# wuxiyang1996/iPLAN

Hardware: AMD Instinct MI355X
Metric: env-steps/sec (whole node), Hetero-Highway chaotic 5-agent (higher is better)
Workload: dtype f32; 1 GPU; Highway chaotic full iPLAN (Behaviour + GAT + soft update), 5 agents x 55 entities, 32 envs/GPU x 90 steps; step = 8 rollouts, each followed by insert + Behavior_policy.learn + Prediction_policy.learn, then IPPOLearner.train (15 epochs x 255 x 90 rows x 5 agents); envs_per_gpu=32

## Files before the change

iplan_amd/csrc/behavior_learn.hip:

```cpp
#define IPLAN_SPLIT_PAIRS
#include <cstdlib>

#include "api_util.h"
#include "gru_tile.h"

namespace iplan {

constexpr int DHd = 64, DT = 4;
constexpr int EHd = 32, ET = 2;
constexpr int DLD = DHd + 8;
constexpr int ELDB = EHd + 8;
constexpr int SVD = IPLAN_BEH_SAVE_DEC, SVE = IPLAN_BEH_SAVE_ENC, SVL = IPLAN_BEH_SAVE_LAT;
constexpr int DSD = IPLAN_BEH_DSAVE_DEC, DSL = IPLAN_BEH_DSAVE_LAT;
constexpr float BEPS = 1e-10f;
constexpr int DEC_FWD_BIAS = 64 + 192 + 192 + 16;
constexpr int SD_X = 0, SD_U = 32, SD_R = 96, SD_Z = 160, SD_N = 224, SD_HN = 288, SD_H = 352, SD_A = 416, SD_Y = 480;
constexpr int DD_DY = 0, DD_DU = 16, DD_DR = 80, DD_DZ = 144, DD_DNI = 208, DD_DNH = 272;
constexpr int SE_U = 0, SE_R = 32, SE_Z = 64, SE_N = 96, SE_HN = 128, SE_H = 160;

__device__ __forceinline__ float chain_sum_b(float v) {
    v += __shfl_xor(v, 1);
    v += __shfl_xor(v, 2);
    v += __shfl_xor(v, 4);
    v += __shfl_xor(v, 8);
    return v;
}

__device__ __forceinline__ int beh_windows(const IplanBehArgs& a) { return a.hard ? a.T / a.L - 1 : a.T - 1 - a.L; }
__device__ __forceinline__ int beh_x_step(const IplanBehArgs& a, int j, int t) { return a.hard ? j * a.L + t : j - (a.L - 1) + t; }
__device__ __forceinline__ int beh_y_step(const IplanBehArgs& a, int j, int t) { return a.hard ? (j + 1) * a.L + t : j + 1 + t; }
__device__ __forceinline__ int beh_m_step(const IplanBehArgs& a, int j, int t) { return a.hard ? j * a.L + t : j + 1 + t; }

__device__ __forceinline__ uint32_t keep_hash(uint64_t seed, uint64_t idx) {
    uint32_t x = (uint32_t)idx ^ ((uint32_t)(idx >> 32) * 0x9E3779B9u) ^ (uint32_t)seed;
    x ^= x >> 16; x *= 0x85EBCA6Bu; x ^= x >> 13; x *= 0xC2B2AE35u; x ^= x >> 16;
    x ^= (uint32_t)(seed >> 32);
    x ^= x >> 15; x *= 0x2C1B3C6Du; x ^= x >> 12;
    return x;
}
__device__ __forceinline__ f32x4 keep_flags4(uint64_t seed, uint64_t base, float p) {
    const uint32_t thr = (uint32_t)(p * 65536.0f);
    const uint32_t h0 = keep_hash(seed, base), h1 = keep_hash(seed, base + 2);
    f32x4 k;
    k[0] = (h0 & 0xFFFFu) >= thr ? 1.0f : 0.0f;
    k[1] = (h0 >> 16) >= thr ? 1.0f : 0.0f;
    k[2] = (h1 & 0xFFFFu) >= thr ? 1.0f : 0.0f;
    k[3] = (h1 >> 16) >= thr ? 1.0f : 0.0f;
    return k;
}

__device__ __forceinline__ f32x4 keep_tile(const IplanBehArgs& a, int net, int j, int row, int t, int T, bool valid, int rows) {
    const int l = lane_id(), g = l >> 4;
    const int64_t base = ((((int64_t)net * beh_windows(a) + j) * rows + row) * a.L + t) * DHd + 16 * T + 4 * g;
    f32x4 k = splat4(0.f);
    if (!valid) return k;
    if (a.keep) {
        for (int q = 0; q < 4; ++q) k[q] = (float)a.keep[base + q];
    } else if (a.drop_p > 0.f) {
        k = keep_flags4(a.seed, (uint64_t)base, a.drop_p);
    } else {
        k = splat4(1.0f);
    }
    return k;
}

__device__ __forceinline__ float window_mask_sum(const IplanBehArgs& a, int net, int j) {
    if (a.win_norm) return a.win_norm[(int64_t)net * beh_windows(a) + j] * (float)(a.N * a.d);
    float s = 0.f;
    const int span = a.hard ? beh_windows(a) * a.L : a.L;
    const int first = a.hard ? 0 : j + 1;
    const int cnt = a.E * span;
    for (int i = lane_id(); i < cnt; i += 64) {
        const int e = i / span, t = i - e * span;
        s += a.mask[((int64_t)net * a.E + e) * a.T + first + t];
    }
    return wave_sum(s) * (float)(a.N * a.d);
}

__device__ __forceinline__ f32x4 ld_row_raw(const float* __restrict__ row, int dim, int g) {
    f32x4 v;
    for (int q = 0; q < 4; ++q) {
        const int i = 4 * g + q;
        v[q] = row[i < dim ? i : dim - 1];
    }
    return v;
}
struct BehChain {
    int net, rows, tiles, tile, row, e, ent, J, n, g;
    bool valid;
    const float* hrow;
    const float* mrow;
    int64_t grow;
};
__device__ __forceinline__ bool beh_chain(const IplanBehArgs& a, BehChain& c) {
    const int l = lane_id();
    c.n = l & 15;
    c.g = l >> 4;
    c.net = (int)blockIdx.y;
    c.rows = a.E * a.N;
    c.tiles = (c.rows + 15) / 16;
    c.tile = (int)blockIdx.x * 4 + (wave_id() & 3);
    c.row = c.tile * 16 + c.n;
    c.valid = c.tile < c.tiles && c.row < c.rows;
    c.e = c.valid ? c.row / a.N : 0;
    c.ent = c.valid ? c.row % a.N : 0;
    c.J = beh_windows(a);
    c.hrow = a.hist ? a.hist + (int64_t)c.net * a.h_s_net + (int64_t)c.e * a.h_s_e + (int64_t)c.ent * a.d : nullptr;
    c.mrow = a.mask ? a.mask + ((int64_t)c.net * a.E + c.e) * a.T : nullptr;
    c.grow = (int64_t)c.net * c.rows + (c.valid ? c.row : 0);
    return c.tile < c.tiles;
}

template <bool BF3>
__global__ __launch_bounds__(256) void beh_enc_fwd_kernel(IplanBehArgs a) {
    __shared__ __attribute__((aligned(16))) float s_wih[BF3 ? 16 : 3 * EHd * ELDB];
    __shared__ __attribute__((aligned(16))) float s_whh[BF3 ? 16 : 3 * EHd * ELDB];
    __shared__ __attribute__((aligned(16))) float s_lin[EHd * 24];
    __shared__ __attribute__((aligned(16))) float s_out[16 * ELDB];
    __shared__ __attribute__((aligned(16))) float s_b[32 + 96 + 96 + 16];
    const float* __restrict__ PE = a.enc_params + (int64_t)blockIdx.y * a.enc_s_net;
    if (!BF3) {
        stage_matrix(s_wih, ELDB, 3 * EHd, PE + a.enc_off[IPLAN_ENC_WIH], 3 * EHd, EHd);
        stage_matrix(s_whh, ELDB, 3 * EHd, PE + a.enc_off[IPLAN_ENC_WHH], 3 * EHd, EHd);
    }
    stage_matrix(s_lin, 24, EHd, PE + a.enc_off[IPLAN_ENC_LIN_W], EHd, a.d);
    stage_matrix(s_out, ELDB, 16, PE + a.enc_off[IPLAN_ENC_OUT_W], a.Z, EHd);
    stage_vector(s_b, 32, PE + a.enc_off[IPLAN_ENC_LIN_B], 32);
    stage_vector(s_b + 32, 96, PE + a.enc_off[IPLAN_ENC_BIH], 96);
    stage_vector(s_b + 128, 96, PE + a.enc_off[IPLAN_ENC_BHH], 96);
    stage_vector(s_b + 224, 16, PE + a.enc_off[IPLAN_ENC_OUT_B], a.Z);
    __syncthreads();
    BehChain c;
    if (!beh_chain(a, c)) return;
    const bool valid = c.valid;
    const int g = c.g, J = c.J, l = lane_id();
    const int j_lo = imax(a.fwd_j_lo, 0), j_hi = a.fwd_j_hi > 0 ? imin(a.fwd_j_hi, J) : J;
    float* carry = a.enc_carry ? a.enc_carry + ((int64_t)c.net * c.tiles + c.tile) * 768 : nullptr;
    f32x4 he[ET], lat = splat4(0.f);
    for (int t = 0; t < ET; ++t) he[t] = splat4(0.f);
    if (j_lo > 0 && carry) {
        for (int t = 0; t < ET; ++t) he[t] = *reinterpret_cast<const f32x4*>(carry + 256 * t + 4 * l);
        lat = *reinterpret_cast<const f32x4*>(carry + 512 + 4 * l);
    }
    auto x_fetch = [&](int j, int t, bool& has) {
        const int st = beh_x_step(a, j, t);
        has = st >= 0;
        return ld_row_raw(c.hrow + (int64_t)(st < 0 ? 0 : st) * a.h_s_t, a.d, g);
    };
    bool x_has = false;
    f32x4 x_raw = x_fetch(j_lo, 0, x_has);
    const int64_t ecgs = (int64_t)J * a.L * 256;
    float* enc_rec = a.saved_enc + ((int64_t)c.net * c.tiles + (c.tile < c.tiles ? c.tile : 0)) * (SVE / 16) * ecgs + 16 * c.n;
    Bf3 wih[BF3 ? 6 : 1], whh[BF3 ? 6 : 1];
    f32x4 b_rz[4], b_in[2], b_hn[2];
    if (BF3) {
        for (int t = 0; t < 6; ++t) {
            wih[t] = wfrag_bf3(PE + a.enc_off[IPLAN_ENC_WIH], EHd, 3 * EHd, 16 * t, 0);
            whh[t] = wfrag_bf3(PE + a.enc_off[IPLAN_ENC_WHH], EHd, 3 * EHd, 16 * t, 0);
        }
        for (int t = 0; t < 4; ++t) b_rz[t] = bfrag_lds(s_b + 32, t) + bfrag_lds(s_b + 128, t);
        for (int t = 0; t < 2; ++t) { b_in[t] = bfrag_lds(s_b + 32, 4 + t); b_hn[t] = bfrag_lds(s_b + 128, 4 + t); }
    }
    for (int j = j_lo; j < j_hi; ++j) {
        float* sl = a.saved_lat + (c.grow * J + j) * SVL;
        vstore_a(sl + 16, valid, 0, lat);
        for (int t = 0; t < a.L; ++t) {
            f32x4 x1[1];
            for (int q = 0; q < 4; ++q) x1[0][q] = keep_if(valid && x_has && 4 * g + q < a.d, x_raw[q]);
            {
                const bool last_t = t + 1 == a.L, more = j + 1 < j_hi;
                x_raw = x_fetch(last_t && more ? j + 1 : j, last_t ? (more ? 0 : t) : t + 1, x_has);
            }
            float* se = enc_rec + ((int64_t)j * a.L + t) * 256;
            f32x4 ue[ET];
            for (int T = 0; T < ET; ++T) {
                ue[T] = relu4(dense_tile<1>(s_lin, 24, 16 * T, x1, bfrag_lds(s_b, T)));
                vstore_a(se + ((SE_U >> 4) + T) * ecgs, valid, 0, ue[T]);
            }
            GruGates ke[ET];
            if (BF3) {
                const Bf3 us = split_bf3(ue[0], ue[1]), hs = split_bf3(he[0], he[1]);
                f32x4 acc[6] = {b_rz[0], b_rz[1], b_rz[2], b_rz[3], b_in[0], b_in[1]}, ahn[2] = {b_hn[0], b_hn[1]};
#define ENC_BF3_ROUND(WP, XP)                                                          \
    for (int cc = 0; cc < 6; ++cc) acc[cc] = mfma_bf16(wih[cc].WP, us.XP, acc[cc]);
                ENC_BF3_ROUND(p2, p0) ENC_BF3_ROUND(p0, p2) ENC_BF3_ROUND(p1, p1) ENC_BF3_ROUND(p1, p0) ENC_BF3_ROUND(p0, p1) ENC_BF3_ROUND(p0, p0)
#undef ENC_BF3_ROUND
#define ENC_BF3_ROUND(WP, XP)                                                          \
    for (int cc = 0; cc < 4; ++cc) acc[cc] = mfma_bf16(whh[cc].WP, hs.XP, acc[cc]);    \
    for (int cc = 0; cc < 2; ++cc) ahn[cc] = mfma_bf16(whh[4 + cc].WP, hs.XP, ahn[cc]);
                ENC_BF3_ROUND(p2, p0) ENC_BF3_ROUND(p0, p2) ENC_BF3_ROUND(p1, p1) ENC_BF3_ROUND(p1, p0) ENC_BF3_ROUND(p0, p1) ENC_BF3_ROUND(p0, p0)
#undef ENC_BF3_ROUND
                for (int T = 0; T < ET; ++T) {
                    ke[T] = gru_gates(acc[T], acc[2 + T], acc[4 + T], ahn[T], he[T]);
                    he[T] = ke[T].h;
                }
            } else {
                gru_step_lds<ET, ET>(s_wih, ELDB, s_whh, ELDB, s_b + 32, s_b + 128, ue, he, ke);
            }
            for (int T = 0; T < ET; ++T) {
                vstore_a(se + ((SE_R >> 4) + T) * ecgs, valid, 0, ke[T].r);
                vstore_a(se + ((SE_Z >> 4) + T) * ecgs, valid, 0, ke[T].z);
                vstore_a(se + ((SE_N >> 4) + T) * ecgs, valid, 0, ke[T].n);
                vstore_a(se + ((SE_HN >> 4) + T) * ecgs, valid, 0, ke[T].hn);
                vstore_a(se + ((SE_H >> 4) + T) * ecgs, valid, 0, he[T]);
            }
        }
        const f32x4 lg = dense_tile<ET>(s_out, ELDB, 0, he, bfrag_lds(s_b + 224, 0));
        float mx = -INFINITY;
        for (int q = 0; q < 4; ++q)
            if (4 * g + q < a.Z) mx = fmaxf(mx, lg[q]);
        mx = fmaxf(mx, __shfl_xor(mx, 16));
        mx = fmaxf(mx, __shfl_xor(mx, 32));
        f32x4 ex;
        float ss = 0.f;
        for (int q = 0; q < 4; ++q) { ex[q] = (4 * g + q < a.Z) ? expf(lg[q] - mx) : 0.f; ss += ex[q]; }
        ss = group_sum(ss);
        f32x4 nl;
        for (int q = 0; q < 4; ++q) nl[q] = ex[q] / ss;
        vstore_a(sl, valid, 0, nl);
        for (int q = 0; q < 4; ++q) lat[q] = a.hard ? nl[q] : (1.0f - a.coef) * lat[q] + nl[q] * a.coef;
    }
    if (j_hi < J && carry) {
        for (int t = 0; t < ET; ++t) *reinterpret_cast<f32x4*>(carry + 256 * t + 4 * l) = he[t];
        *reinterpret_cast<f32x4*>(carry + 512 + 4 * l) = lat;
    }
}

constexpr int DEC_TILES = 3;
constexpr int DEC_THREADS = 256 * DEC_TILES;


struct DecTile {
    int net, rows, tiles, tile, J;
    bool live, full, valid;
    int n, g, row, e, ent;
    uint32_t rec_lane;
    const char* hist;
    uint32_t hist_lane;
    const char* mask;
    uint32_t mask_lane;
    int64_t grow0;
    int64_t trow0;
};
__device__ __forceinline__ void dec_tile(const IplanBehArgs& a, DecTile& c, int tile) {
    const int l = lane_id();
    c.n = l & 15;
    c.g = l >> 4;
    c.net = (int)blockIdx.y;
    c.rows = a.E * a.N;
    c.tiles = (c.rows + 15) / 16;
    c.tile = tile;
    c.live = tile < c.tiles;
    c.full = c.live && tile * 16 + 15 < c.rows;
    c.row = tile * 16 + c.n;
    c.valid = c.live && c.row < c.rows;
    const int rr = c.valid ? c.row : 0;
    c.e = rr / a.N;
    c.ent = rr - c.e * a.N;
    c.J = beh_windows(a);
    c.hist = reinterpret_cast<const char*>(a.hist ? a.hist + (int64_t)c.net * a.h_s_net : nullptr);
    c.hist_lane = (uint32_t)(((int64_t)c.e * a.h_s_e + (int64_t)c.ent * a.d) * 4);
    c.mask = reinterpret_cast<const char*>(a.mask ? a.mask + (int64_t)c.net * a.E * a.T : nullptr);
    c.mask_lane = (uint32_t)(c.e * a.T * 4);
    c.grow0 = (int64_t)c.net * c.rows + (int64_t)(c.live ? tile : 0) * 16;
    c.trow0 = ((int64_t)c.net * c.tiles + (int64_t)(c.live ? tile : 0)) * 16;
}

#define REC_CG(col) ((uint32_t)((col) >> 4))

template <bool FULL>
__device__ __forceinline__ f32x4 ld4(const char* __restrict__ base, uint32_t off, bool valid) {
    const f32x4 v = *reinterpret_cast<const f32x4*>(base + ((FULL || valid) ? off : 0u));
    return FULL ? v : zero_unless(valid, v);
}
template <bool FULL>
__device__ __forceinline__ f32x4 ld4_raw(const char* __restrict__ base, uint32_t off, bool valid) {
    return *reinterpret_cast<const f32x4*>(base + ((FULL || valid) ? off : 0u));
}
template <bool FULL>
__device__ __forceinline__ f32x4 ld_row_raw(const char* __restrict__ base, uint32_t off, bool valid, int dim, int g) {
    const uint32_t o = (FULL || valid) ? off : 0u;
    f32x4 v;
    for (int q = 0; q < 4; ++q) {
        const int i = 4 * g + q;
        v[q] = *reinterpret_cast<const float*>(base + (o + 4u * (uint32_t)(i < dim ? i : dim - 1)));
    }
    return v;
}
template <bool FULL>
__device__ __forceinline__ void st4(char* __restrict__ base, uint32_t off, bool valid, f32x4 v) {
    if (FULL || valid) *reinterpret_cast<f32x4*>(base + off) = v;
}
template <bool FULL>
__device__ __forceinline__ f32x4 ld_row_br(const char* __restrict__ base, uint32_t off, bool valid, int dim, int g) {
    f32x4 v = splat4(0.f);
    if (FULL || valid) {
        const float* p = reinterpret_cast<const float*>(base + off) + 4 * g;
        for (int q = 0; q < 4; ++q)
            if (4 * g + q < dim) v[q] = p[q];
    }
    return v;
}

constexpr int XF_H = 0, XF_U = 4, XF_Y = 8, XF_SLOTS = 11;

template <bool FULL, int Q>
__device__ __forceinline__ void dec_fwd_body(const IplanBehArgs& a, const DecTile& c, const float* __restrict__ s_wih,
                                             const float* __restrict__ s_whh, const float* __restrict__ s_lin,
                                             const float* __restrict__ s_out, const float* __restrict__ s_b, float* __restrict__ xch,
                                             int* __restrict__ tcnt) {
    constexpr int q = Q;
#ifndef DEC_FWD_TILE_SYNC
#define DEC_FWD_TILE_SYNC 0
#endif
#ifndef DEC_BWD_TILE_SYNC
#define DEC_BWD_TILE_SYNC 1
#endif
    int sync_n = 0;
    auto tile_sync = [&]() {
        if (DEC_FWD_TILE_SYNC) { sync_n += 4; IPLAN_TILE_SYNC(tcnt, sync_n); }
        else IPLAN_LDS_BARRIER();
    };
    const bool valid = c.valid;
    const int l = lane_id(), g = c.g, J = c.J, net = c.net;
    const float inv_keep = 1.0f / (1.0f - a.drop_p);
    const bool dec_only = a.win != nullptr;
    const int Lw = a.L;
    auto put = [&](int slot, f32x4 v) { *reinterpret_cast<f32x4*>(xch + slot * 256 + 4 * l) = v; };
    auto get = [&](int slot) { return *reinterpret_cast<const f32x4*>(xch + slot * 256 + 4 * l); };
    const int j_lo = dec_only ? 0 : imax(a.fwd_j_lo, 0), j_hi = (!dec_only && a.fwd_j_hi > 0) ? imin(a.fwd_j_hi, J) : J;
    const int64_t steps_per_chain = (int64_t)J * Lw;
    char* sd_base = reinterpret_cast<char*>(a.saved_dec + c.trow0 * steps_per_chain * SVD);
    const uint32_t sd_lane = 64u * (uint32_t)c.n + 16u * (uint32_t)g, cgs = (uint32_t)(steps_per_chain * 1024);
    const char* sl_base = reinterpret_cast<const char*>(a.saved_lat ? a.saved_lat + c.grow0 * J * SVL : nullptr);
    const uint32_t sl_lane = (uint32_t)((int64_t)c.n * J * SVL * 4);
    float* carry = (a.dec_carry && c.live) ? a.dec_carry + ((int64_t)net * c.tiles + c.tile) * 1024 : nullptr;
    const int64_t grow = c.grow0 + c.n;

    auto latent_shifted = [&](int j) {
        f32x4 v = splat4(0.f);
        if (FULL || valid) {
            const float* lp = dec_only ? a.lat_in + grow * a.Z
                                       : reinterpret_cast<const float*>(sl_base + sl_lane + (uint32_t)j * (uint32_t)(SVL * 4)) + 16;
            for (int k = 0; k < 4; ++k) {
                const int z = 4 * g + k - a.d;
                if (z >= 0 && z < a.Z) v[k] = lp[z];
            }
        }
        return v;
    };
    auto x_of = [&](int j, int t) {
        if (dec_only) return ld_row_br<FULL>(reinterpret_cast<const char*>(a.win), (uint32_t)((grow * Lw + t) * a.d * 4), valid, a.d, g);
        const int st = beh_x_step(a, j, t);
        if (st < 0) return splat4(0.f);
        return ld_row_br<FULL>(c.hist, c.hist_lane + (uint32_t)((int64_t)st * a.h_s_t * 4), valid, a.d, g);
    };
    auto u_own = [&](f32x4 xin) {
        f32x4 x1[1];
        x1[0] = xin;
        return relu4(dense_tile<1>(s_lin, 24, 16 * q, x1, bfrag_lds(s_b, q)));
    };

    f32x4 h[DT], u[DT];
    for (int i = 0; i < DT; ++i) h[i] = dec_only ? ld4<FULL>(reinterpret_cast<const char*>(a.hd_in), (uint32_t)(grow * DHd * 4) + 64u * i + 16u * g, valid)
                                                 : splat4(0.f);
    if (j_lo > 0 && carry)
        for (int i = 0; i < DT; ++i) h[i] = *reinterpret_cast<const f32x4*>(carry + 256 * i + 4 * l);
    f32x4 latsh = latent_shifted(j_lo);
    f32x4 xin = x_of(j_lo, 0) + latsh;
    put(XF_U + q, u_own(xin));
    tile_sync();
    for (int i = 0; i < DT; ++i) u[i] = get(XF_U + i);
    tile_sync();

    float beh = 0.f, stab = 0.f;
    const int rows3[3] = {16 * q, DHd + 16 * q, 2 * DHd + 16 * q};
    for (int j = j_lo; j < j_hi; ++j) {
        const float scale = (dec_only || q) ? 0.f : (float)(a.d * a.N) / (window_mask_sum(a, net, j) + BEPS);
        float err = 0.f;
        f32x4 latsh_next = latsh;
        if (j + 1 < j_hi) latsh_next = latent_shifted(j + 1);
        for (int t = 0; t < Lw; ++t) {
            const uint32_t so = sd_lane + (uint32_t)(((int64_t)j * Lw + t) * 1024);
            const bool last_t = t + 1 == Lw;
            const bool has_next = !last_t || j + 1 < j_hi;
            f32x4 xin_next = splat4(0.f);
            if (has_next) xin_next = x_of(last_t ? j + 1 : j, last_t ? 0 : t + 1) + (last_t ? latsh_next : latsh);
            f32x4 nx = splat4(0.f);
            float m = 0.f;
            if (q == 0 && !dec_only) {
                nx = ld_row_br<FULL>(c.hist, c.hist_lane + (uint32_t)((int64_t)beh_y_step(a, j, t) * a.h_s_t * 4), valid, a.d, g);
                if (FULL || valid) m = *reinterpret_cast<const float*>(c.mask + c.mask_lane + 4u * (uint32_t)beh_m_step(a, j, t));
            }
            if (q == 0) st4<FULL>(sd_base, so + cgs * REC_CG(SD_X), valid, xin);
            st4<FULL>(sd_base, so + cgs * REC_CG(SD_U + 16 * q), valid, u[q]);
            f32x4 ai[3], ah[3];
            ai[0] = bfrag_lds(s_b + 64, q) + bfrag_lds(s_b + 256, q);
            ai[1] = bfrag_lds(s_b + 64, DT + q) + bfrag_lds(s_b + 256, DT + q);
            ai[2] = bfrag_lds(s_b + 64, 2 * DT + q);
            dense_multi<3, DT>(s_wih, DLD, rows3, 0, u, ai);
            ah[0] = ai[0];
            ah[1] = ai[1];
            ah[2] = bfrag_lds(s_b + 256, 2 * DT + q);
            dense_multi<3, DT>(s_whh, DLD, rows3, 0, h, ah);
            const GruGates o = gru_gates(ah[0], ah[1], ai[2], ah[2], h[q]);
            st4<FULL>(sd_base, so + cgs * REC_CG(SD_R + 16 * q), valid, o.r);
            st4<FULL>(sd_base, so + cgs * REC_CG(SD_Z + 16 * q), valid, o.z);
            st4<FULL>(sd_base, so + cgs * REC_CG(SD_N + 16 * q), valid, o.n);
            st4<FULL>(sd_base, so + cgs * REC_CG(SD_HN + 16 * q), valid, o.hn);
            st4<FULL>(sd_base, so + cgs * REC_CG(SD_H + 16 * q), valid, o.h);
            const f32x4 km = keep_tile(a, net, j, c.row, t, q, FULL || valid, c.rows);
            f32x4 act[1];
            for (int k = 0; k < 4; ++k) act[0][k] = tanh_f(o.h[k]) * (km[k] * inv_keep);
            st4<FULL>(sd_base, so + cgs * REC_CG(SD_A + 16 * q), valid, act[0]);
            const f32x4 yp = dense_tile_k<1>(s_out, DLD, 0, 16 * q, act, q ? splat4(0.f) : bfrag_lds(s_b + 448, 0));
            put(XF_H + q, o.h);
            if (q) put(XF_Y + q - 1, yp);
            if (has_next) put(XF_U + q, u_own(xin_next));
            tile_sync();
            for (int i = 0; i < DT; ++i) h[i] = (i == q) ? o.h : get(XF_H + i);
            if (has_next)
                for (int i = 0; i < DT; ++i) u[i] = get(XF_U + i);
            f32x4 y = yp;
            if (q == 0) y = (yp + get(XF_Y)) + (get(XF_Y + 1) + get(XF_Y + 2));
            tile_sync();
            const f32x4 xt = xin;
            xin = xin_next;
            if (q) continue;
            st4<FULL>(sd_base, so + cgs * REC_CG(SD_Y), valid, y);
            if (dec_only) {
                if (FULL || valid) {
                    float* po = a.pred_out + (grow * Lw + t) * a.d + 4 * g;
                    for (int k = 0; k < 4; ++k)
                        if (4 * g + k < a.d) po[k] = y[k];
                }
                continue;
            }
            float d2 = 0.f;
            for (int k = 0; k < 4; ++k) {
                if (4 * g + k < a.d) {
                    err += fabsf(nx[k] - y[k]) * m;
                    const float df = xt[k] - y[k];
                    d2 = fmaf(df, df, d2);
                }
            }
            d2 = group_sum(d2);
            if ((FULL || valid) && g == 0) stab += fmaxf(sqrtf(d2) - a.thres, 0.f);
        }
        latsh = latsh_next;
        if (dec_only) {
            st4<FULL>(reinterpret_cast<char*>(a.hd_out), (uint32_t)(grow * DHd * 4) + 64u * q + 16u * g, valid, h[q]);
            return;
        }
        beh = fmaf(err, scale, beh);
    }
    if (j_hi < J && carry) *reinterpret_cast<f32x4*>(carry + 256 * q + 4 * l) = h[q];
    beh = chain_sum_b(group_sum(beh)) / (a.hard ? 1.0f : (float)J);
    stab = chain_sum_b(group_sum(stab)) / (float)a.E / (float)a.L / (float)J;
    if (l == 0 && q == 0 && c.live) {
        float* lp = a.loss_part + ((int64_t)net * c.tiles + c.tile) * 2;
        lp[0] = j_lo > 0 ? lp[0] + beh : beh;
        lp[1] = j_lo > 0 ? lp[1] + stab : stab;
    }
}

__global__ __launch_bounds__(DEC_THREADS) void beh_dec_fwd_kernel(IplanBehArgs a) {
    IPLAN_DYN_LDS(smem);
    float* s_wih = smem;
    float* s_whh = s_wih + 3 * DHd * DLD;
    float* s_lin = s_whh + 3 * DHd * DLD;
    float* s_out = s_lin + DHd * 24;
    float* s_b = s_out + 16 * DLD;
    float* s_xch = s_b + DEC_FWD_BIAS;
    int* s_tcnt = reinterpret_cast<int*>(s_xch + DEC_TILES * XF_SLOTS * 256);
    if (threadIdx.x < 16) s_tcnt[threadIdx.x] = 0;
    const float* __restrict__ PD = a.dec_params + (int64_t)blockIdx.y * a.dec_s_net;
    stage_matrix(s_wih, DLD, 3 * DHd, PD + a.dec_off[IPLAN_DEC_WIH], 3 * DHd, DHd);
    stage_matrix(s_whh, DLD, 3 * DHd, PD + a.dec_off[IPLAN_DEC_WHH], 3 * DHd, DHd);
    stage_matrix(s_lin, 24, DHd, PD + a.dec_off[IPLAN_DEC_LIN_W], DHd, a.d + a.Z);
    stage_matrix(s_out, DLD, 16, PD + a.dec_off[IPLAN_DEC_OUT_W], a.d, DHd);
    stage_vector(s_b, 64, PD + a.dec_off[IPLAN_DEC_LIN_B], 64);
    stage_vector(s_b + 64, 192, PD + a.dec_off[IPLAN_DEC_BIH], 192);
    stage_vector(s_b + 256, 192, PD + a.dec_off[IPLAN_DEC_BHH], 192);
    stage_vector(s_b + 448, 16, PD + a.dec_off[IPLAN_DEC_OUT_B], a.d);
    __syncthreads();
    const int w = uniform_i(wave_id()), q = w & 3, ts = w >> 2;
    DecTile c;
    dec_tile(a, c, (int)blockIdx.x * DEC_TILES + ts);
    float* xch = s_xch + ts * (XF_SLOTS * 256);
#define IPLAN_DEC_FWD(F, QQ) dec_fwd_body<F, QQ>(a, c, s_wih, s_whh, s_lin, s_out, s_b, xch, s_tcnt + ts)
    if (c.full) { if (q == 0) IPLAN_DEC_FWD(true, 0); else if (q == 1) IPLAN_DEC_FWD(true, 1); else if (q == 2) IPLAN_DEC_FWD(true, 2); else IPLAN_DEC_FWD(true, 3); }
    else { if (q == 0) IPLAN_DEC_FWD(false, 0); else if (q == 1) IPLAN_DEC_FWD(false, 1); else if (q == 2) IPLAN_DEC_FWD(false, 2); else IPLAN_DEC_FWD(false, 3); }
#undef IPLAN_DEC_FWD
}

__global__ __launch_bounds__(64) void beh_loss_kernel(IplanBehArgs a) {
    const int net = (int)blockIdx.x;
    const int tiles = (a.E * a.N + 15) / 16;
    float b = 0.f, s = 0.f;
    for (int i = lane_id(); i < tiles; i += 64) {
        b += a.loss_part[((int64_t)net * tiles + i) * 2];
        s += a.loss_part[((int64_t)net * tiles + i) * 2 + 1];
    }
    b = wave_sum(b);
    s = wave_sum(s);
    if (lane_id() == 0) {
        a.loss[net * 2] = b;
        a.loss[net * 2 + 1] = s;
    }
}

constexpr int XB_SLOTS = 16;

template <bool FULL, int Q>
__device__ __forceinline__ void dec_bwd_body(const IplanBehArgs& a, const DecTile& c, const float* __restrict__ s_wihT,
                                             const float* __restrict__ s_whhT, const float* __restrict__ s_outT,
                                             const float* __restrict__ s_latT, float* __restrict__ xch, int* __restrict__ tcnt) {
    constexpr int TLD = 3 * DHd + 8;
    int sync_n = 0;
    auto tile_sync = [&]() {
        if (DEC_BWD_TILE_SYNC) { sync_n += 4; IPLAN_TILE_SYNC(tcnt, sync_n); }
        else IPLAN_LDS_BARRIER();
    };
    const bool valid = c.valid;
    const int l = lane_id(), g = c.g, J = c.J, net = c.net, Lw = a.L;
    const float inv_keep = 1.0f / (1.0f - a.drop_p);
    auto put = [&](int slot, f32x4 v) { *reinterpret_cast<f32x4*>(xch + slot * 256 + 4 * l) = v; };
    auto get = [&](int slot) { return *reinterpret_cast<const f32x4*>(xch + slot * 256 + 4 * l); };
    const int64_t steps_per_chain = (int64_t)J * Lw;
    const char* sd_base = reinterpret_cast<const char*>(a.saved_dec + c.trow0 * steps_per_chain * SVD);
    const uint32_t sd_lane = 64u * (uint32_t)c.n + 16u * (uint32_t)g, cgs = (uint32_t)(steps_per_chain * 1024);
    char* dd_base = reinterpret_cast<char*>(a.dsave_dec + c.trow0 * steps_per_chain * DSD);
    const uint32_t dd_lane = sd_lane;
    char* dl_base = reinterpret_cast<char*>(a.dsave_lat + c.grow0 * J * DSL);
    const uint32_t dl_lane = (uint32_t)((int64_t)c.n * J * DSL * 4) + 16u * (uint32_t)g;

    struct StepIn {
        f32x4 r, z, n, hn, hp, u, y, nx, xc;
        float m;
        bool first, has_xc;
    };
    auto load_step = [&](int j, int t, StepIn& o) {
        const uint32_t so = sd_lane + (uint32_t)(((int64_t)j * Lw + t) * 1024);
        o.first = (j == 0 && t == 0);
        o.r = ld4_raw<FULL>(sd_base, so + cgs * REC_CG(SD_R + 16 * Q), valid);
        o.z = ld4_raw<FULL>(sd_base, so + cgs * REC_CG(SD_Z + 16 * Q), valid);
        o.n = ld4_raw<FULL>(sd_base, so + cgs * REC_CG(SD_N + 16 * Q), valid);
        o.hn = ld4_raw<FULL>(sd_base, so + cgs * REC_CG(SD_HN + 16 * Q), valid);
        o.u = ld4_raw<FULL>(sd_base, so + cgs * REC_CG(SD_U + 16 * Q), valid);
        o.hp = ld4_raw<FULL>(sd_base, (o.first ? so : so - 1024u) + cgs * REC_CG(SD_H + 16 * Q), valid);
        o.y = ld4_raw<FULL>(sd_base, so + cgs * REC_CG(SD_Y), valid);
        o.nx = ld_row_raw<FULL>(c.hist, c.hist_lane + (uint32_t)((int64_t)beh_y_step(a, j, t) * a.h_s_t * 4), valid, a.d, g);
        o.m = *reinterpret_cast<const float*>(c.mask + c.mask_lane + 4u * (uint32_t)beh_m_step(a, j, t));
        o.has_xc = false;
        o.xc = splat4(0.f);
        if (a.penalty != 0.f) {
            const int st = beh_x_step(a, j, t);
            o.has_xc = st >= 0;
            o.xc = ld_row_raw<FULL>(c.hist, c.hist_lane + (uint32_t)((int64_t)(st < 0 ? 0 : st) * a.h_s_t * 4), valid, a.d, g);
        }
    };
    auto mask_step = [&](StepIn& o) {
        o.hp = zero_unless(!o.first, o.hp);
        for (int k = 0; k < 4; ++k) o.xc[k] = keep_if(o.has_xc && 4 * g + k < a.d, o.xc[k]);
        if (!FULL) {
            o.r = zero_unless(valid, o.r); o.z = zero_unless(valid, o.z); o.n = zero_unless(valid, o.n);
            o.hn = zero_unless(valid, o.hn); o.u = zero_unless(valid, o.u); o.hp = zero_unless(valid, o.hp);
            o.y = zero_unless(valid, o.y); o.nx = zero_unless(valid, o.nx); o.xc = zero_unless(valid, o.xc);
            o.m = keep_if(valid, o.m);
        }
    };
    const float pen = a.penalty / (float)J / (float)(a.E_norm > 0 ? a.E_norm : a.E) / (float)Lw;
    const int j_hi = a.bwd_j_hi > 0 ? imin(a.bwd_j_hi, J) : J, j_lo = imax(a.bwd_j_lo, 0);
    float* carry = (a.dec_carry && c.live) ? a.dec_carry + ((int64_t)net * c.tiles + c.tile) * 1024 + 256 * Q : nullptr;
    f32x4 dhd = (j_hi < J && carry) ? *reinterpret_cast<const f32x4*>(carry + 4 * l) : splat4(0.f);
    StepIn cur;
    load_step(j_hi - 1, Lw - 1, cur);
    f32x4 hcur = ld4<FULL>(sd_base, sd_lane + (uint32_t)((((int64_t)(j_hi - 1)) * Lw + (Lw - 1)) * 1024) + cgs * REC_CG(SD_H + 16 * Q), valid);
    for (int j = j_hi - 1; j >= j_lo; --j) {
        const float scale = (float)(a.d * a.N) / (window_mask_sum(a, net, j) + BEPS) / (a.hard ? 1.0f : (float)J);
        f32x4 dlat = splat4(0.f);
        for (int t = Lw - 1; t >= 0; --t) {
            const uint32_t dof = dd_lane + (uint32_t)(((int64_t)j * Lw + t) * 1024);
            mask_step(cur);
            f32x4 dy[1];
            for (int k = 0; k < 4; ++k) {
                float v = 0.f;
                if ((FULL || valid) && 4 * g + k < a.d) {
                    const float er = cur.nx[k] - cur.y[k];
                    v = -((er > 0.f) ? 1.0f : (er < 0.f ? -1.0f : 0.0f)) * cur.m * scale;
                }
                dy[0][k] = v;
            }
            if (a.penalty != 0.f) {
                float d2 = 0.f;
                f32x4 df;
                for (int k = 0; k < 4; ++k) {
                    df[k] = (4 * g + k < a.d) ? cur.xc[k] - cur.y[k] : 0.f;
                    d2 = fmaf(df[k], df[k], d2);
                }
                const float nrm = sqrtf(group_sum(d2));
                if ((FULL || valid) && nrm > a.thres)
                    for (int k = 0; k < 4; ++k) dy[0][k] -= pen * df[k] / nrm;
            }
#ifndef BWD_ABL
#define BWD_ABL 0
#endif
            if (Q == 0 && BWD_ABL != 1) st4<FULL>(dd_base, dof + cgs * REC_CG(DD_DY), valid, dy[0]);
            const f32x4 da = dense_tile<1>(s_outT, 24, 16 * Q, dy, splat4(0.f));
            const f32x4 km = keep_tile(a, net, j, c.row, t, Q, FULL || valid, c.rows);
            f32x4 dht;
            for (int k = 0; k < 4; ++k) {
                const float th = tanh_f(hcur[k]);
                dht[k] = fmaf(da[k] * km[k] * inv_keep, 1.0f - th * th, dhd[k]);
            }
            const GruGrads o = gru_gates_bwd(dht, cur.r, cur.z, cur.n, cur.hn, cur.hp);
            if (BWD_ABL != 1) {
                st4<FULL>(dd_base, dof + cgs * REC_CG(DD_DR + 16 * Q), valid, o.dr);
                st4<FULL>(dd_base, dof + cgs * REC_CG(DD_DZ + 16 * Q), valid, o.dz);
                st4<FULL>(dd_base, dof + cgs * REC_CG(DD_DNI + 16 * Q), valid, o.dni);
                st4<FULL>(dd_base, dof + cgs * REC_CG(DD_DNH + 16 * Q), valid, o.dnh);
            }
            put(0 * 4 + Q, o.dr);
            put(1 * 4 + Q, o.dz);
            put(2 * 4 + Q, o.dni);
            put(3 * 4 + Q, o.dnh);
            const f32x4 u_own = cur.u;
            hcur = cur.hp;
            IPLAN_SCHED_FENCE();
            if (BWD_ABL != 2) {
                const bool wrap = t == 0, more = j > j_lo;
                load_step(wrap && more ? j - 1 : j, wrap ? (more ? Lw - 1 : 0) : t - 1, cur);
            }
            if (BWD_ABL != 5) tile_sync();
            f32x4 du = splat4(0.f), pd = splat4(0.f);
            auto b_ih = [&](int kt) { const int gate = kt >> 2, T = kt & 3;
                                      return (T == Q) ? (gate == 0 ? o.dr : (gate == 1 ? o.dz : o.dni)) : get(gate * 4 + T); };
            auto b_hn = [&](int T) { return (T == Q) ? o.dnh : get(3 * 4 + T); };
            f32x4 fa = wfrag_lds(s_wihT, TLD, 16 * Q, 0), fb = wfrag_lds(s_whhT, TLD, 16 * Q, 0);
            f32x4 bi = b_ih(0), bh = bi;
#pragma unroll
            for (int kt = 0; kt < 3 * DT; ++kt) {
                f32x4 fan = fa, fbn = fb, bin = bi, bhn = bh;
                if (kt + 1 < 3 * DT) {
                    fan = wfrag_lds(s_wihT, TLD, 16 * Q, 16 * (kt + 1));
                    fbn = wfrag_lds(s_whhT, TLD, 16 * Q, 16 * (kt + 1));
                    bin = b_ih(kt + 1);
                    bhn = (kt + 1) < 2 * DT ? bin : b_hn((kt + 1) & 3);
                }
                if (BWD_ABL != 3)
                    for (int k = 0; k < 4; ++k) {
                        du = mfma4(fa[k], bi[k], du);
                        pd = mfma4(fb[k], bh[k], pd);
                    }
                else { du += fa * bi; pd += fb * bh; }
                fa = fan; fb = fbn; bi = bin; bh = bhn;
            }
            f32x4 dup[1];
            for (int k = 0; k < 4; ++k) dup[0][k] = u_own[k] > 0.f ? du[k] : 0.f;
            if (BWD_ABL != 1) st4<FULL>(dd_base, dof + cgs * REC_CG(DD_DU + 16 * Q), valid, dup[0]);
            dhd = o.dh_direct + pd;
            dlat = dense_tile_k<1>(s_latT, DLD, 0, 16 * Q, dup, dlat);
            if (BWD_ABL != 4) tile_sync();
        }
        if (Q) put(Q - 1, dlat);
        tile_sync();
        if (Q == 0) st4<FULL>(dl_base, dl_lane + (uint32_t)j * (uint32_t)(DSL * 4), valid, (dlat + get(0)) + (get(1) + get(2)));
        tile_sync();
    }
    if (j_lo > 0 && carry) *reinterpret_cast<f32x4*>(carry + 4 * l) = dhd;
}

__global__ __launch_bounds__(DEC_THREADS) void beh_dec_bwd_kernel(IplanBehArgs a) {
    IPLAN_DYN_LDS(smem);
    constexpr int TLD = 3 * DHd + 8;
    float* s_wihT = smem;
    float* s_whhT = s_wihT + DHd * TLD;
    float* s_outT = s_whhT + DHd * TLD;
    float* s_latT = s_outT + DHd * 24;
    float* s_xch = s_latT + 16 * DLD;
    int* s_tcnt = reinterpret_cast<int*>(s_xch + DEC_TILES * XB_SLOTS * 256);
    if (threadIdx.x < 16) s_tcnt[threadIdx.x] = 0;
    const float* __restrict__ PD = a.dec_params + (int64_t)blockIdx.y * a.dec_s_net;
    const int din = a.d + a.Z;
    stage_matrix_t(s_wihT, TLD, DHd, PD + a.dec_off[IPLAN_DEC_WIH], 3 * DHd, DHd);
    stage_matrix_t(s_whhT, TLD, DHd, PD + a.dec_off[IPLAN_DEC_WHH], 3 * DHd, DHd);
    stage_matrix_t(s_outT, 24, DHd, PD + a.dec_off[IPLAN_DEC_OUT_W], a.d, DHd);
    {
        const float* Wl = PD + a.dec_off[IPLAN_DEC_LIN_W];
        for (int idx = (int)threadIdx.x; idx < 16 * DLD; idx += (int)blockDim.x) {
            const int z = idx / DLD, m = idx - z * DLD;
            s_latT[idx] = (z < a.Z && m < DHd) ? Wl[(int64_t)m * din + a.d + z] : 0.f;
        }
    }
    __syncthreads();
    const int w = uniform_i(wave_id()), q = w & 3, ts = w >> 2;
    DecTile c;
    dec_tile(a, c, (int)blockIdx.x * DEC_TILES + ts);
    float* xch = s_xch + ts * (XB_SLOTS * 256);
#define IPLAN_DEC_BWD(F, QQ) dec_bwd_body<F, QQ>(a, c, s_wihT, s_whhT, s_outT, s_latT, xch, s_tcnt + ts)
    if (c.full) { if (q == 0) IPLAN_DEC_BWD(true, 0); else if (q == 1) IPLAN_DEC_BWD(true, 1); else if (q == 2) IPLAN_DEC_BWD(true, 2); else IPLAN_DEC_BWD(true, 3); }
    else { if (q == 0) IPLAN_DEC_BWD(false, 0); else if (q == 1) IPLAN_DEC_BWD(false, 1); else if (q == 2) IPLAN_DEC_BWD(false, 2); else IPLAN_DEC_BWD(false, 3); }
#undef IPLAN_DEC_BWD
}

constexpr int EP_WIH = 0, EP_WHH = 3072, EP_BIH = 6144, EP_BHH = 6240, EP_LINW = 6336, EP_LINB = 6848, EP_OUTW = 6880, EP_OUTB = 7392;
static_assert(IPLAN_BEH_ENC_PART == 7408, "enc_part layout");

constexpr int EB_FRAGS = 2 * 2 * 3;
template <bool BF3>
__global__ __launch_bounds__(256) void beh_enc_bwd_kernel(IplanBehArgs a) {
    constexpr int TLE = 3 * EHd + 8;
    __shared__ __attribute__((aligned(16))) float s_wihT[BF3 ? 16 : EHd * TLE];
    __shared__ __attribute__((aligned(16))) float s_whhT[BF3 ? 16 : EHd * TLE];
    __shared__ __attribute__((aligned(16))) bf16x8 s_wp[BF3 ? EB_FRAGS * 3 * 64 : 1];
    __shared__ __attribute__((aligned(16))) float s_outT[EHd * 24];
    __shared__ __attribute__((aligned(16))) float s_turn[4][15][256];
    const float* __restrict__ PE = a.enc_params + (int64_t)blockIdx.y * a.enc_s_net;
    if (BF3) {
        for (int f = wave_id(); f < EB_FRAGS; f += 4) {
            const int mtx = f / 6, T = (f / 3) & 1, ch = f % 3;
            const Bf3 w = wfrag_t_bf3(PE + a.enc_off[mtx ? IPLAN_ENC_WHH : IPLAN_ENC_WIH], EHd, 16 * T, 32 * ch);
            s_wp[(f * 3 + 0) * 64 + lane_id()] = w.p0;
            s_wp[(f * 3 + 1) * 64 + lane_id()] = w.p1;
            s_wp[(f * 3 + 2) * 64 + lane_id()] = w.p2;
        }
    } else {
        stage_matrix_t(s_wihT, TLE, EHd, PE + a.enc_off[IPLAN_ENC_WIH], 3 * EHd, EHd);
        stage_matrix_t(s_whhT, TLE, EHd, PE + a.enc_off[IPLAN_ENC_WHH], 3 * EHd, EHd);
    }
    stage_matrix_t(s_outT, 24, EHd, PE + a.enc_off[IPLAN_ENC_OUT_W], a.Z, EHd);
    __syncthreads();
    BehChain c;
    const bool live = beh_chain(a, c);
    const bool valid = c.valid;
    const int l = lane_id(), n = c.n, g = c.g, J = c.J;
    float (*turn)[256] = s_turn[wave_id()];
    const float cn = a.hard ? 1.0f : a.coef, ck = a.hard ? 0.0f : 1.0f - a.coef;

    f32x4 aWih[6][2], aWhh[6][2], aLin[2], aOut[2];
    f32x4 bG[8], bU[2], bO;
    for (int t = 0; t < 6; ++t)
        for (int u = 0; u < 2; ++u) { aWih[t][u] = splat4(0.f); aWhh[t][u] = splat4(0.f); }
    for (int u = 0; u < 2; ++u) { aLin[u] = splat4(0.f); aOut[u] = splat4(0.f); bU[u] = splat4(0.f); }
    for (int t = 0; t < 8; ++t) bG[t] = splat4(0.f);
    bO = splat4(0.f);
    auto park = [&](int slot, f32x4 v) { *reinterpret_cast<f32x4*>(&turn[slot][n * 16 + ((4 * g + 4 * (n >> 1)) & 15)]) = v; };
    auto pick = [&](int slot, int s) { const int r = 4 * s + g; return turn[slot][r * 16 + ((n + 4 * (r >> 1)) & 15)]; };

    const int j_hi = a.bwd_j_hi > 0 ? imin(a.bwd_j_hi, J) : J, j_lo = imax(a.bwd_j_lo, 0);
    float* carry = (a.enc_carry && live) ? a.enc_carry + ((int64_t)c.net * c.tiles + c.tile) * 768 : nullptr;
    f32x4 dhe[ET], dlat = splat4(0.f);
    for (int t = 0; t < ET; ++t) dhe[t] = splat4(0.f);
    if (j_hi < J && carry) {
        for (int t = 0; t < ET; ++t) dhe[t] = *reinterpret_cast<const f32x4*>(carry + 256 * t + 4 * l);
        dlat = *reinterpret_cast<const f32x4*>(carry + 512 + 4 * l);
    }
    struct EncIn {
        f32x4 r[ET], z[ET], n[ET], hn[ET], u[ET], hp[ET], x;
        bool first, has_x;
    };
    const bool ok = valid && live;
    const int64_t ecgs = (int64_t)J * a.L * 256;
    const float* rec0 = a.saved_enc + ((int64_t)c.net * c.tiles + (c.tile < c.tiles ? c.tile : 0)) * (SVE / 16) * ecgs + 16 * c.n + 4 * g;
    auto load_step = [&](int j, int t, EncIn& o) {
        const int64_t step = (int64_t)j * a.L + t;
        o.first = step == 0;
        const float* se = rec0 + step * 256;
        const float* sp = o.first ? se : se - 256;
        for (int T = 0; T < ET; ++T) {
            o.hp[T] = *reinterpret_cast<const f32x4*>(sp + ((SE_H >> 4) + T) * ecgs);
            o.u[T] = *reinterpret_cast<const f32x4*>(se + ((SE_U >> 4) + T) * ecgs);
            o.r[T] = *reinterpret_cast<const f32x4*>(se + ((SE_R >> 4) + T) * ecgs);
            o.z[T] = *reinterpret_cast<const f32x4*>(se + ((SE_Z >> 4) + T) * ecgs);
            o.n[T] = *reinterpret_cast<const f32x4*>(se + ((SE_N >> 4) + T) * ecgs);
            o.hn[T] = *reinterpret_cast<const f32x4*>(se + ((SE_HN >> 4) + T) * ecgs);
        }
        const int st = beh_x_step(a, j, t);
        o.has_x = st >= 0;
        o.x = ld_row_raw(c.hrow + (int64_t)(st < 0 ? 0 : st) * a.h_s_t, a.d, g);
    };
    auto mask_step = [&](EncIn& o) {
        for (int T = 0; T < ET; ++T) {
            o.hp[T] = zero_unless(ok && !o.first, o.hp[T]);
            o.u[T] = zero_unless(ok, o.u[T]);
            o.r[T] = zero_unless(ok, o.r[T]);
            o.z[T] = zero_unless(ok, o.z[T]);
            o.n[T] = zero_unless(ok, o.n[T]);
            o.hn[T] = zero_unless(ok, o.hn[T]);
        }
        for (int q = 0; q < 4; ++q) o.x[q] = keep_if(ok && o.has_x && 4 * g + q < a.d, o.x[q]);
    };
    struct WinIn {
        f32x4 nl, dl, hL[ET];
    };
    auto load_win = [&](int j, WinIn& o) {
        o.nl = *reinterpret_cast<const f32x4*>(a.saved_lat + (c.grow * J + j) * SVL + 4 * g);
        o.dl = *reinterpret_cast<const f32x4*>(a.dsave_lat + (c.grow * J + j) * DSL + 4 * g);
        for (int T = 0; T < ET; ++T) o.hL[T] = *reinterpret_cast<const f32x4*>(rec0 + ((int64_t)j * a.L + (a.L - 1)) * 256 + ((SE_H >> 4) + T) * ecgs);
    };
    EncIn cur;
    WinIn win;
    load_step(j_hi - 1, a.L - 1, cur);
    load_win(j_hi - 1, win);
    for (int j = j_hi - 1; j >= j_lo; --j) {
        f32x4 dlog[1], hL[ET];
        {
            const f32x4 nl = zero_unless(ok && a.Z > 1, win.nl);
            float s = 0.f;
            f32x4 dnew;
            for (int q = 0; q < 4; ++q) { dnew[q] = cn * dlat[q]; s = fmaf(nl[q], dnew[q], s); }
            s = group_sum(s);
            const f32x4 dl_dec = zero_unless(ok, win.dl);
            for (int q = 0; q < 4; ++q) {
                dlog[0][q] = nl[q] * (dnew[q] - s);
                dlat[q] = ck * dlat[q] + dl_dec[q];
                bO[q] += dlog[0][q];
            }
            for (int T = 0; T < ET; ++T) {
                hL[T] = zero_unless(ok, win.hL[T]);
                dhe[T] = dense_tile<1>(s_outT, 24, 16 * T, dlog, dhe[T]);
            }
            park(0, dlog[0]); park(1, hL[0]); park(2, hL[1]);
            IPLAN_WAVE_SYNC();
            for (int s4 = 0; s4 < 4; ++s4) {
                const float av = pick(0, s4);
                aOut[0] = mfma4(av, pick(1, s4), aOut[0]);
                aOut[1] = mfma4(av, pick(2, s4), aOut[1]);
            }
            IPLAN_WAVE_SYNC();
        }
        for (int t = a.L - 1; t >= 0; --t) {
            f32x4 dg[4 * ET], dd[ET], u[ET], hp[ET];
            mask_step(cur);
            for (int T = 0; T < ET; ++T) {
                hp[T] = cur.hp[T];
                u[T] = cur.u[T];
                const GruGrads o = gru_gates_bwd(dhe[T], cur.r[T], cur.z[T], cur.n[T], cur.hn[T], hp[T]);
                dg[T] = o.dr; dg[ET + T] = o.dz; dg[2 * ET + T] = o.dni; dg[3 * ET + T] = o.dnh;
                dd[T] = o.dh_direct;
            }
            for (int k = 0; k < 8; ++k) bG[k] += dg[k];
            const int oe[ET] = {0, 16};
            f32x4 du[ET], dup[ET];
            for (int T = 0; T < ET; ++T) { du[T] = splat4(0.f); dhe[T] = dd[T]; }
            if (BF3) {
                for (int ch = 0; ch < 3; ++ch) {
                    const Bf3 gi = split_bf3(dg[2 * ch], dg[2 * ch + 1]);
                    const Bf3 gh = ch < 2 ? gi : split_bf3(dg[3 * ET], dg[3 * ET + 1]);
                    Bf3 wi[ET], wh[ET];
                    for (int T = 0; T < ET; ++T) {
                        const bf16x8* fi = s_wp + ((0 * 2 + T) * 3 + ch) * 3 * 64 + l;
                        const bf16x8* fh = s_wp + ((1 * 2 + T) * 3 + ch) * 3 * 64 + l;
                        wi[T].p0 = fi[0]; wi[T].p1 = fi[64]; wi[T].p2 = fi[128];
                        wh[T].p0 = fh[0]; wh[T].p1 = fh[64]; wh[T].p2 = fh[128];
                    }
#define ENCB_ROUND(WP, XP)                                                           \
    for (int T = 0; T < ET; ++T) {                                                   \
        du[T] = mfma_bf16(wi[T].WP, gi.XP, du[T]);                                   \
        dhe[T] = mfma_bf16(wh[T].WP, gh.XP, dhe[T]);                                 \
    }
                    ENCB_ROUND(p2, p0) ENCB_ROUND(p0, p2) ENCB_ROUND(p1, p1) ENCB_ROUND(p1, p0) ENCB_ROUND(p0, p1) ENCB_ROUND(p0, p0)
#undef ENCB_ROUND
                }
            } else {
                dense_multi<ET, 3 * ET>(s_wihT, TLE, oe, 0, dg, du);
                dense_multi<ET, 2 * ET>(s_whhT, TLE, oe, 0, dg, dhe);
                dense_multi<ET, ET>(s_whhT, TLE, oe, 2 * EHd, dg + 3 * ET, dhe);
            }
            for (int T = 0; T < ET; ++T) {
                for (int q = 0; q < 4; ++q) dup[T][q] = u[T][q] > 0.f ? du[T][q] : 0.f;
                bU[T] += dup[T];
            }
            for (int k = 0; k < 8; ++k) park(k, dg[k]);
            park(8, dup[0]); park(9, dup[1]); park(10, u[0]); park(11, u[1]); park(12, hp[0]); park(13, hp[1]); park(14, cur.x);
            IPLAN_SCHED_FENCE();
            {
                const bool wrap = t == 0, more = j > j_lo;
                load_step(wrap && more ? j - 1 : j, wrap ? (more ? a.L - 1 : 0) : t - 1, cur);
                if (wrap) load_win(more ? j - 1 : j, win);
            }
            IPLAN_WAVE_SYNC();
            for (int s4 = 0; s4 < 4; ++s4) {
                const float u0 = pick(10, s4), u1 = pick(11, s4), h0 = pick(12, s4), h1 = pick(13, s4), xv = pick(14, s4);
                for (int o = 0; o < 6; ++o) {
                    const float ai = pick(o, s4);
                    const float ah = o < 4 ? ai : pick(o + 2, s4);
                    aWih[o][0] = mfma4(ai, u0, aWih[o][0]);
                    aWih[o][1] = mfma4(ai, u1, aWih[o][1]);
                    aWhh[o][0] = mfma4(ah, h0, aWhh[o][0]);
                    aWhh[o][1] = mfma4(ah, h1, aWhh[o][1]);
                }
                aLin[0] = mfma4(pick(8, s4), xv, aLin[0]);
                aLin[1] = mfma4(pick(9, s4), xv, aLin[1]);
            }
            IPLAN_WAVE_SYNC();
        }
    }
    if (!live) return;
    if (j_lo > 0 && carry) {
        for (int t = 0; t < ET; ++t) *reinterpret_cast<f32x4*>(carry + 256 * t + 4 * l) = dhe[t];
        *reinterpret_cast<f32x4*>(carry + 512 + 4 * l) = dlat;
    }
    const bool add = j_hi < J;
    float* part = a.enc_part + ((int64_t)c.net * c.tiles + c.tile) * IPLAN_BEH_ENC_PART;
    auto put_part = [&](int idx, float v) { part[idx] = add ? part[idx] + v : v; };
    for (int o = 0; o < 6; ++o)
        for (int u = 0; u < 2; ++u)
            for (int q = 0; q < 4; ++q) {
                const int orow = 16 * o + 4 * g + q, col = 16 * u + n;
                put_part(EP_WIH + orow * EHd + col, aWih[o][u][q]);
                put_part(EP_WHH + orow * EHd + col, aWhh[o][u][q]);
            }
    for (int u = 0; u < 2; ++u)
        for (int q = 0; q < 4; ++q) {
            put_part(EP_LINW + (16 * u + 4 * g + q) * 16 + n, aLin[u][q]);
            put_part(EP_OUTW + (4 * g + q) * EHd + 16 * u + n, aOut[u][q]);
        }
    for (int k = 0; k < 8; ++k)
        for (int q = 0; q < 4; ++q) {
            const float sum = chain_sum_b(bG[k][q]);
            if (n == 0) {
                const int gate = k >> 1, T = k & 1, idx = 16 * T + 4 * g + q;
                if (gate < 3) put_part(EP_BIH + gate * EHd + idx, sum);
                if (gate < 2) put_part(EP_BHH + gate * EHd + idx, sum);
                if (gate == 3) put_part(EP_BHH + 2 * EHd + idx, sum);
            }
        }
    for (int T = 0; T < 2; ++T)
        for (int q = 0; q < 4; ++q) {
            const float sum = chain_sum_b(bU[T][q]);
            if (n == 0) put_part(EP_LINB + 16 * T + 4 * g + q, sum);
        }
    for (int q = 0; q < 4; ++q) {
        const float sum = chain_sum_b(bO[q]);
        if (n == 0) put_part(EP_OUTB + 4 * g + q, sum);
    }
}

__global__ __launch_bounds__(256) void beh_enc_grad_kernel(IplanBehArgs a) {
    const int net = (int)blockIdx.y;
    const int tiles = (a.E * a.N + 15) / 16;
    const int idx = (int)(blockIdx.x * blockDim.x + threadIdx.x);
    const int sizes[8] = {EHd * a.d, EHd, 3 * EHd * EHd, 3 * EHd * EHd, 3 * EHd, 3 * EHd, a.Z * EHd, a.Z};
    int rem = idx, which = -1;
    for (int k = 0; k < 8; ++k) {
        if (rem < sizes[k]) { which = k; break; }
        rem -= sizes[k];
    }
    if (which < 0) return;
    int src;
    switch (which) {
        case IPLAN_ENC_LIN_W: src = EP_LINW + (rem / a.d) * 16 + rem % a.d; break;
        case IPLAN_ENC_LIN_B: src = EP_LINB + rem; break;
        case IPLAN_ENC_WIH: src = EP_WIH + rem; break;
        case IPLAN_ENC_WHH: src = EP_WHH + rem; break;
        case IPLAN_ENC_BIH: src = EP_BIH + rem; break;
        case IPLAN_ENC_BHH: src = EP_BHH + rem; break;
        case IPLAN_ENC_OUT_W: src = EP_OUTW + rem; break;
        default: src = EP_OUTB + rem; break;
    }
    const float* part = a.enc_part + (int64_t)net * tiles * IPLAN_BEH_ENC_PART + src;
    float s = 0.f;
    for (int t = 0; t < tiles; ++t) s += part[(int64_t)t * IPLAN_BEH_ENC_PART];
    float* dst = a.enc_grad + (int64_t)net * a.enc_grad_s_net + a.enc_off[which] + rem;
    *dst = a.enc_grad_beta != 0.f ? fmaf(a.enc_grad_beta, *dst, s) : s;
}

typedef __bf16 bf16x4 __attribute__((ext_vector_type(4)));
constexpr int D2_TILES = 3, D2_THREADS = 512, D2_LAG = 2;
constexpr int D2_GI = D2_TILES * 4 * 2 * 3 * 256;
constexpr int D2_HX = D2_TILES * 2 * 2 * 3 * 256;
constexpr int D2_UX = D2_HX;
constexpr int D2_YX = D2_TILES * 2 * 4 * 128;
constexpr int D2_CNT_INTS = 20;
constexpr int D2_MAX_WINDOWS = 512;
constexpr int D2_LDS_FLOATS = D2_GI + D2_HX + D2_UX + D2_YX + D2_CNT_INTS + D2_MAX_WINDOWS;

typedef int i32x4 __attribute__((ext_vector_type(4)));
#ifdef IPLAN_HOST_EMULATION
__device__ inline void d2_signal(int* c) { IPLAN_WAVE_SYNC(); if (lane_id() == 0) *c += 1; }
__device__ inline void d2_wait(const int* c, int target) { while (*reinterpret_cast<const volatile int*>(c) < target) iplan_emu::yield_(); }
__device__ inline void d2_wait4(const int* c, int target, int live) {
    for (;;) {
        bool ok = true;
        for (int i = 0; i < 4; ++i) ok = ok && (!((live >> i) & 1) || reinterpret_cast<const volatile int*>(c)[i] >= target);
        if (ok) return;
        iplan_emu::yield_();
    }
}
#else
__device__ __forceinline__ void d2_signal(int* c) {
    asm volatile("s_waitcnt lgkmcnt(0)" ::: "memory");
    if ((threadIdx.x & 63u) == 0) __hip_atomic_fetch_add(c, 1, __ATOMIC_RELAXED, __HIP_MEMORY_SCOPE_WORKGROUP);
}
__device__ __forceinline__ void d2_wait(const int* c, int target) {
    while (__hip_atomic_load(c, __ATOMIC_RELAXED, __HIP_MEMORY_SCOPE_WORKGROUP) < target) __builtin_amdgcn_s_sleep(1);
    asm volatile("" ::: "memory");
}
__device__ __forceinline__ void d2_wait4(const int* c, int target, int live) {
    const i32x4 dead = {(live & 1) ? 0 : 0x7fffffff, (live & 2) ? 0 : 0x7fffffff, (live & 4) ? 0 : 0x7fffffff, (live & 8) ? 0 : 0x7fffffff};
    for (;;) {
        const i32x4 v = *reinterpret_cast<const volatile i32x4*>(c) | dead;
        const int lo = min(min(v[0], v[1]), min(v[2], v[3]));
        if (__builtin_amdgcn_readfirstlane(lo) >= target) break;
        __builtin_amdgcn_s_sleep(1);
    }
    asm volatile("" ::: "memory");
}
#endif

__device__ __forceinline__ void split_bf3_half(f32x4 v, bf16x4& p0, bf16x4& p1, bf16x4& p2) {
    u32x2 q0, q1, q2;
    for (int k = 0; k < 2; ++k) {
        f32x2 w;
        w[0] = v[2 * k];
        w[1] = v[2 * k + 1];
        uint32_t a, b, c;
        split_bf3_pair(w, a, b, c);
        q0[k] = a; q1[k] = b; q2[k] = c;
    }
    p0 = __builtin_bit_cast(bf16x4, q0);
    p1 = __builtin_bit_cast(bf16x4, q1);
    p2 = __builtin_bit_cast(bf16x4, q2);
}
__device__ __forceinline__ void d2_contract(const Bf3 (&W)[3][2], const Bf3 (&x)[2], f32x4 (&acc)[3]) {
#define D2_ROUND(WP, XP)                     \
    for (int cc = 0; cc < 2; ++cc)           \
        for (int gt = 0; gt < 3; ++gt) acc[gt] = mfma_bf16(W[gt][cc].WP, x[cc].XP, acc[gt]);
    D2_ROUND(p2, p0) D2_ROUND(p0, p2) D2_ROUND(p1, p1) D2_ROUND(p1, p0) D2_ROUND(p0, p1) D2_ROUND(p0, p0)
#undef D2_ROUND
}

#ifndef D2_ABL
#define D2_ABL 0
#endif
#if defined(D2_CLOCKS) && !defined(IPLAN_HOST_EMULATION)
__device__ long long g_d2_clk[32];
#define D2_CLK_DECL(n) long long clk_acc[n]; for (int ci = 0; ci < n; ++ci) clk_acc[ci] = 0; long long clk_last = __builtin_amdgcn_s_memtime(); const bool clk_on = blockIdx.x == 0 && blockIdx.y == 0 && q == 0
#define D2_CLK(i) do { if (clk_on) { const long long now = __builtin_amdgcn_s_memtime(); clk_acc[i] += now - clk_last; clk_last = now; } } while (0)
#define D2_CLK_OUT(base, n) do { if (clk_on && l == 0) for (int ci = 0; ci < n; ++ci) g_d2_clk[base + ci] = clk_acc[ci]; } while (0)
#else
#define D2_CLK_DECL(n) do {} while (0)
#define D2_CLK(i) do {} while (0)
#define D2_CLK_OUT(base, n) do {} while (0)
#endif

constexpr int D2_VM_WINDOW = 16;
#ifdef IPLAN_HOST_EMULATION
__device__ inline void d2_gload(float& dst, const char* sbase, uint32_t voff) { dst = *reinterpret_cast<const float*>(sbase + voff); }
__device__ inline const char* d2_ubase(const char* p) { return p; }
template <int WINDOW> __device__ inline void d2_landed(float (&)[4], float (&)[4]) {}
template <int WINDOW> __device__ inline void d2_landed(float (&)[4], float (&)[4], float&) {}
__device__ inline void d2_drain_vm() {}
#else
__device__ __forceinline__ void d2_gload(float& dst, const char* sbase, uint32_t voff) {
    asm volatile("global_load_dword %0, %1, %2" : "=v"(dst) : "v"(voff), "s"(sbase) : "memory");
}
__device__ __forceinline__ const char* d2_ubase(const char* p) {
    const uint64_t b = reinterpret_cast<uint64_t>(p);
    const uint32_t lo = __builtin_amdgcn_readfirstlane((uint32_t)b), hi = __builtin_amdgcn_readfirstlane((uint32_t)(b >> 32));
    const char* u = reinterpret_cast<const char*>(((uint64_t)hi << 32) | lo);
    asm volatile("s_nop 4" : "+s"(u));
    return u;
}
template <int WINDOW> __device__ __forceinline__ void d2_landed(float (&a)[4], float (&b)[4]) {
    asm volatile("s_waitcnt vmcnt(%8)" : "+v"(a[0]), "+v"(a[1]), "+v"(a[2]), "+v"(a[3]), "+v"(b[0]), "+v"(b[1]), "+v"(b[2]), "+v"(b[3]) : "n"(WINDOW) : "memory");
}
template <int WINDOW> __device__ __forceinline__ void d2_landed(float (&a)[4], float (&b)[4], float& m) {
    asm volatile("s_waitcnt vmcnt(%9)" : "+v"(a[0]), "+v"(a[1]), "+v"(a[2]), "+v"(a[3]), "+v"(b[0]), "+v"(b[1]), "+v"(b[2]), "+v"(b[3]), "+v"(m) : "n"(WINDOW) : "memory");
}
__device__ __forceinline__ void d2_drain_vm() { asm volatile("s_waitcnt vmcnt(0)" ::: "memory"); }
#endif

struct D2Ctx {
    float *s_gi, *s_hx, *s_ux, *s_yx, *s_scale;
    int *hcnt, *ucnt, *ycnt, *rcnt, *gcnt, *bcnt;
    int q, l, n, g, net, J, Lw, j_lo, j_hi, steps, YL, n_live;
    int64_t steps_per_chain;
    uint32_t cgs;
    const float* PD;
};
__device__ __forceinline__ void d2_px_write(const D2Ctx& x, float* base, int k, int par, f32x4 v) {
    bf16x4 p0, p1, p2;
    split_bf3_half(v, p0, p1, p2);
    char* slot = reinterpret_cast<char*>(base + ((k * 2 + par) * 2 + (x.q >> 1)) * 3 * 256) + 16 * x.l + 8 * (x.q & 1);
    *reinterpret_cast<bf16x4*>(slot) = p0;
    *reinterpret_cast<bf16x4*>(slot + 1024) = p1;
    *reinterpret_cast<bf16x4*>(slot + 2048) = p2;
}
__device__ __forceinline__ void d2_px_read(const D2Ctx& x, const float* base, int k, int par, Bf3 (&v)[2]) {
    for (int cc = 0; cc < 2; ++cc) {
        const char* slot = reinterpret_cast<const char*>(base + ((k * 2 + par) * 2 + cc) * 3 * 256) + 16 * x.l;
        v[cc].p0 = *reinterpret_cast<const bf16x8*>(slot);
        v[cc].p1 = *reinterpret_cast<const bf16x8*>(slot + 1024);
        v[cc].p2 = *reinterpret_cast<const bf16x8*>(slot + 2048);
    }
}
__device__ __forceinline__ f32x4* d2_gi_slot(const D2Ctx& x, int k, int slot, int gate) {
    return reinterpret_cast<f32x4*>(x.s_gi + (((k * 4 + x.q) * 2 + slot) * 3 + gate) * 256) + x.l;
}
__device__ __forceinline__ char* d2_sd_base(const IplanBehArgs& a, const D2Ctx& x, const DecTile& ct) {
    return reinterpret_cast<char*>(a.saved_dec + ct.trow0 * x.steps_per_chain * SVD);
}
__device__ __forceinline__ uint32_t d2_sd_off(const D2Ctx& x, int step) {
    return 64u * (uint32_t)x.n + 16u * (uint32_t)x.g + (uint32_t)((int64_t)step * 1024);
}

template <bool FAST, bool SAVE_ACT>
__device__ __forceinline__ void d2_recurrent(const IplanBehArgs& a, const D2Ctx& x, const DecTile (&c)[D2_TILES]) {
    const int q = x.q, l = x.l, g = x.g, net = x.net, Lw = x.Lw;
    (void)g;
    const float* Whh = x.PD + a.dec_off[IPLAN_DEC_WHH];
    Bf3 W[3][2];
    for (int gt = 0; gt < 3; ++gt)
        for (int cc = 0; cc < 2; ++cc) W[gt][cc] = wfrag_bf3(Whh, DHd, 3 * DHd, gt * DHd + 16 * q, 32 * cc);
    const f32x4 bhn = bfrag_a(x.PD + a.dec_off[IPLAN_DEC_BHH], 2 * DT + q);
    const f32x4 wout = wfrag(x.PD + a.dec_off[IPLAN_DEC_OUT_W], DHd, a.d, DHd, 0, 16 * q);
    const f32x4 bout = q ? splat4(0.f) : bfrag(x.PD + a.dec_off[IPLAN_DEC_OUT_B], a.d, 0);
    const float inv_keep = 1.0f / (1.0f - a.drop_p);
    f32x4 hq[D2_TILES];
#pragma unroll
    for (int k = 0; k < D2_TILES; ++k) {
        hq[k] = splat4(0.f);
        if (!FAST && !c[k].live) continue;
        if (x.j_lo > 0 && a.dec_carry)
            hq[k] = *reinterpret_cast<const f32x4*>(a.dec_carry + ((int64_t)net * c[k].tiles + c[k].tile) * 1024 + 256 * q + 4 * l);
        d2_px_write(x, x.s_hx, k, 1, hq[k]);
    }
    d2_signal(x.hcnt);
    int live_mask = 0;
#pragma unroll
    for (int k = 0; k < D2_TILES; ++k) live_mask |= (FAST || c[k].live) ? (1 << k) : 0;
    D2_CLK_DECL(8);
    int j = x.j_lo, t = 0;
    for (int s = 0; s < x.steps; ++s) {
        const uint32_t so = d2_sd_off(x, j * Lw + t);
        D2_CLK(7);
        d2_wait(x.hcnt, 4 * (s + 1));
        d2_wait(x.gcnt, s + 1);
        D2_CLK(0);
        f32x4 acc[D2_TILES][3], gin[D2_TILES];
#pragma unroll
        for (int k = 0; k < D2_TILES; ++k) {
            if (!FAST && !c[k].live) continue;
            Bf3 H[2];
            d2_px_read(x, x.s_hx, k, (s + 1) & 1, H);
            acc[k][0] = *d2_gi_slot(x, k, s & 1, 0);
            acc[k][1] = *d2_gi_slot(x, k, s & 1, 1);
            gin[k] = *d2_gi_slot(x, k, s & 1, 2);
            acc[k][2] = bhn;
            d2_contract(W, H, acc[k]);
        }
        D2_CLK(1);
        d2_signal(x.bcnt);
        GruGates o[D2_TILES];
#pragma unroll
        for (int k = 0; k < D2_TILES; ++k) {
            if (!FAST && !c[k].live) continue;
            o[k] = gru_gates(acc[k][0], acc[k][1], gin[k], acc[k][2], hq[k]);
            hq[k] = o[k].h;
            d2_px_write(x, x.s_hx, k, s & 1, o[k].h);
        }
        d2_signal(x.hcnt);
        D2_CLK(2);
        f32x4 yp[D2_TILES];
#pragma unroll
        for (int k = 0; k < D2_TILES; ++k) {
            if (!FAST && !c[k].live) continue;
            const bool valid = FAST || c[k].valid;
            char* sdb = d2_sd_base(a, x, c[k]);
            if (!(D2_ABL & 1)) {
                st4<FAST>(sdb, so + x.cgs * REC_CG(SD_R + 16 * q), valid, o[k].r);
                st4<FAST>(sdb, so + x.cgs * REC_CG(SD_Z + 16 * q), valid, o[k].z);
                st4<FAST>(sdb, so + x.cgs * REC_CG(SD_N + 16 * q), valid, o[k].n);
                st4<FAST>(sdb, so + x.cgs * REC_CG(SD_HN + 16 * q), valid, o[k].hn);
                st4<FAST>(sdb, so + x.cgs * REC_CG(SD_H + 16 * q), valid, o[k].h);
            }
            const f32x4 km = keep_tile(a, net, j, c[k].row, t, q, valid, c[k].rows);
            f32x4 act;
            for (int i = 0; i < 4; ++i) act[i] = tanh_f(o[k].h[i]) * (km[i] * inv_keep);
            if (SAVE_ACT && !(D2_ABL & 1)) st4<FAST>(sdb, so + x.cgs * REC_CG(SD_A + 16 * q), valid, act);
            yp[k] = mma_block(wout, act, bout);
        }
        D2_CLK(3);
        if (s >= 2) d2_wait4(x.rcnt, s - 1, live_mask);
        D2_CLK(4);
#pragma unroll
        for (int k = 0; k < D2_TILES; ++k)
            if ((FAST || c[k].live) && l < x.YL) *(reinterpret_cast<f32x4*>(x.s_yx + ((k * 2 + (s & 1)) * 4 + q) * 128) + l) = yp[k];
        d2_signal(x.ycnt + q);
        D2_CLK(5);
        if (++t == Lw) { t = 0; ++j; }
    }
    D2_CLK_OUT(0, 8);
#pragma unroll
    for (int k = 0; k < D2_TILES; ++k)
        if ((FAST || c[k].live) && x.j_hi < x.J && a.dec_carry)
            *reinterpret_cast<f32x4*>(a.dec_carry + ((int64_t)net * c[k].tiles + c[k].tile) * 1024 + 256 * q + 4 * l) = hq[k];
}

template <bool FAST, bool Q0>
__device__ __forceinline__ void d2_input(const IplanBehArgs& a, const D2Ctx& x, const DecTile (&c)[D2_TILES]) {
    const int q = x.q, l = x.l, n = x.n, g = x.g, Lw = x.Lw, J = x.J, din = a.d + a.Z;
    const float* Wih = x.PD + a.dec_off[IPLAN_DEC_WIH];
    Bf3 W[3][2];
    for (int gt = 0; gt < 3; ++gt)
        for (int cc = 0; cc < 2; ++cc) W[gt][cc] = wfrag_bf3(Wih, DHd, 3 * DHd, gt * DHd + 16 * q, 32 * cc);
    const float* bih = x.PD + a.dec_off[IPLAN_DEC_BIH];
    const float* bhh = x.PD + a.dec_off[IPLAN_DEC_BHH];
    const f32x4 b_r = bfrag_a(bih, q) + bfrag_a(bhh, q), b_z = bfrag_a(bih, DT + q) + bfrag_a(bhh, DT + q), b_n = bfrag_a(bih, 2 * DT + q);
    const f32x4 wlin = wfrag(x.PD + a.dec_off[IPLAN_DEC_LIN_W], din, DHd, din, 16 * q, 0);
    const f32x4 blin = bfrag_a(x.PD + a.dec_off[IPLAN_DEC_LIN_B], q);
    uint32_t hl[D2_TILES], lv[D2_TILES], vm[D2_TILES], cx[4], cz[4], mx[4], ml[4];
    const char* latb[D2_TILES];
    for (int i = 0; i < 4; ++i) {
        const int col = 4 * g + i, zc = col - a.d;
        mx[i] = col < a.d ? 0xFFFFFFFFu : 0u;
        ml[i] = (zc >= 0 && zc < a.Z) ? 0xFFFFFFFFu : 0u;
        cx[i] = 4u * (uint32_t)(col < a.d ? col : a.d - 1);
        cz[i] = 4u * (uint32_t)(16 + (zc < 0 ? 0 : (zc < a.Z ? zc : a.Z - 1)));
    }
#pragma unroll
    for (int k = 0; k < D2_TILES; ++k) {
        const bool valid = FAST || c[k].valid;
        vm[k] = valid ? 0xFFFFFFFFu : 0u;
        latb[k] = reinterpret_cast<const char*>(a.saved_lat + c[k].grow0 * J * SVL);
        hl[k] = valid ? c[k].hist_lane : 0u;
        lv[k] = (uint32_t)(((int64_t)(valid ? n : 0) * J) * SVL * 4);
    }
    auto bits = [](float v) { return __builtin_bit_cast(uint32_t, v); };
    auto x_fetch4 = [&](float (&v)[4], uint32_t lane_off, int st) {
        const char* hb = d2_ubase(c[0].hist + (int64_t)(st < 0 ? 0 : st) * a.h_s_t * 4);
        for (int i = 0; i < 4; ++i) d2_gload(v[i], hb, lane_off + cx[i]);
    };
    auto lat_fetch4 = [&](float (&v)[4], int k, int jj) {
        const char* lb = d2_ubase(latb[k] + (int64_t)jj * (SVL * 4));
        for (int i = 0; i < 4; ++i) d2_gload(v[i], lb, lv[k] + cz[i]);
    };
    auto x_keep = [&](const float (&v)[4], int st, uint32_t vmask) {
        const uint32_t sm = st >= 0 ? vmask : 0u;
        f32x4 r;
        for (int i = 0; i < 4; ++i) r[i] = __builtin_bit_cast(float, bits(v[i]) & mx[i] & sm);
        return r;
    };
    const int ko = q < D2_TILES ? q : 0;
    DecTile co = c[0];
    if (q == 1) co = c[1];
    if (q == 2) co = c[D2_TILES - 1];
    const bool owner = q < D2_TILES && (FAST || co.live);
    const bool ovalid = FAST || co.valid;
    const uint32_t xoo = q == 1 ? hl[1] : (q == 2 ? hl[D2_TILES - 1] : hl[0]);
    const uint32_t vmo = ovalid ? 0xFFFFFFFFu : 0u;
    float beh = 0.f, stab = 0.f, err = 0.f;
    struct YIn { float nx[4], xt[4], m, scale; };
    auto y_fetch = [&](YIn& o, int jj, int tt) {
        x_fetch4(o.nx, xoo, beh_y_step(a, jj, tt));
        x_fetch4(o.xt, xoo, beh_x_step(a, jj, tt));
        d2_gload(o.m, d2_ubase(co.mask), (ovalid ? co.mask_lane : 0u) + 4u * (uint32_t)beh_m_step(a, jj, tt));
        o.scale = x.s_scale[jj - x.j_lo];
    };
    auto finish_y = [&](int s, int jj, int tt, YIn& in) {
        d2_landed<FAST ? D2_VM_WINDOW : 0>(in.nx, in.xt, in.m);
        d2_wait4(x.ycnt, s + 1, 15);
        f32x4 yq[4];
        for (int i = 0; i < 4; ++i) {
            yq[i] = splat4(0.f);
            if (l < x.YL) yq[i] = *(reinterpret_cast<const f32x4*>(x.s_yx + ((ko * 2 + (s & 1)) * 4 + i) * 128) + l);
        }
        d2_signal(x.rcnt + ko);
        const f32x4 y = (yq[0] + yq[1]) + (yq[2] + yq[3]);
        st4<FAST>(d2_sd_base(a, x, co), d2_sd_off(x, jj * Lw + tt) + x.cgs * REC_CG(SD_Y), ovalid, y);
        const f32x4 nx = x_keep(in.nx, beh_y_step(a, jj, tt), vmo), xt = x_keep(in.xt, beh_x_step(a, jj, tt), vmo);
        const float m = __builtin_bit_cast(float, bits(in.m) & vmo);
        float d2 = 0.f;
        for (int i = 0; i < 4; ++i) {
            const float yi = __builtin_bit_cast(float, bits(y[i]) & mx[i]);
            err += fabsf(nx[i] - yi) * m;
            const float df = xt[i] - yi;
            d2 = fmaf(df, df, d2);
        }
        d2 = group_sum(d2);
        stab += (ovalid && g == 0) ? fmaxf(sqrtf(d2) - a.thres, 0.f) : 0.f;
        if (tt == Lw - 1) { beh = fmaf(err, in.scale, beh); err = 0.f; }
    };
    float xr[D2_TILES][4], lr[D2_TILES][4];
    d2_drain_vm();
#pragma unroll
    for (int k = 0; k < D2_TILES; ++k) {
        x_fetch4(xr[k], hl[k], beh_x_step(a, x.j_lo, 0));
        lat_fetch4(lr[k], k, x.j_lo);
    }
    YIn yin;
    y_fetch(yin, x.j_lo, 0);
    int j = x.j_lo, t = 0, jy = x.j_lo, ty = 0;
    D2_CLK_DECL(8);
    for (int s = 0; s < x.steps; ++s) {
        int jn = j, tn = t + 1;
        if (tn == Lw) { tn = 0; ++jn; }
        if (s + 1 >= x.steps) { jn = j; tn = t; }
        const uint32_t so = d2_sd_off(x, j * Lw + t);
        f32x4 uk[D2_TILES], xk[D2_TILES];
        D2_CLK(7);
#pragma unroll
        for (int k = 0; k < D2_TILES; ++k) {
            if (!FAST && !c[k].live) continue;
            f32x4 xin;
            d2_landed<FAST ? D2_VM_WINDOW : 0>(xr[k], lr[k]);
            {
                const uint32_t sm = beh_x_step(a, j, t) >= 0 ? vm[k] : 0u;
                for (int i = 0; i < 4; ++i) xin[i] = __builtin_bit_cast(float, (bits(xr[k][i]) & mx[i] & sm) | (bits(lr[k][i]) & ml[i] & vm[k]));
            }
            x_fetch4(xr[k], hl[k], beh_x_step(a, jn, tn));
            lat_fetch4(lr[k], k, jn);
            const f32x4 u = relu4(mma_block(wlin, xin, blin));
            uk[k] = u;
            if (Q0) xk[k] = xin;
            d2_px_write(x, x.s_ux, k, s & 1, u);
        }
        d2_signal(x.ucnt);
        D2_CLK(0);
        d2_wait(x.ucnt, 4 * (s + 1));
        D2_CLK(1);
        if (s >= 2) d2_wait(x.bcnt, s - 1);
        D2_CLK(3);
#pragma unroll
        for (int k = 0; k < D2_TILES; ++k) {
            if (!FAST && !c[k].live) continue;
            Bf3 U[2];
            d2_px_read(x, x.s_ux, k, s & 1, U);
            f32x4 acc[3] = {b_r, b_z, b_n};
            d2_contract(W, U, acc);
            *d2_gi_slot(x, k, s & 1, 0) = acc[0];
            *d2_gi_slot(x, k, s & 1, 1) = acc[1];
            *d2_gi_slot(x, k, s & 1, 2) = acc[2];
        }
        D2_CLK(2);
        d2_signal(x.gcnt);
        D2_CLK(4);
        if (!(D2_ABL & 2)) {
#pragma unroll
            for (int k = 0; k < D2_TILES; ++k) {
                if (!FAST && !c[k].live) continue;
                char* sdb = d2_sd_base(a, x, c[k]);
                if (Q0) st4<FAST>(sdb, so + x.cgs * REC_CG(SD_X), FAST || c[k].valid, xk[k]);
                st4<FAST>(sdb, so + x.cgs * REC_CG(SD_U + 16 * q), FAST || c[k].valid, uk[k]);
            }
        }
        if (owner && s >= D2_LAG) {
            finish_y(s - D2_LAG, jy, ty, yin);
            if (++ty == Lw) { ty = 0; ++jy; }
            y_fetch(yin, jy, ty);
        }
        D2_CLK(5);
        if (++t == Lw) { t = 0; ++j; }
    }
    D2_CLK_OUT(8, 8);
    if (!owner) return;
    for (int s = imax(x.steps - D2_LAG, 0); s < x.steps; ++s) {
        d2_drain_vm();
        finish_y(s, jy, ty, yin);
        if (s + 1 < x.steps) {
            if (++ty == Lw) { ty = 0; ++jy; }
            y_fetch(yin, jy, ty);
        }
    }
    d2_drain_vm();
    beh = chain_sum_b(group_sum(beh)) / (a.hard ? 1.0f : (float)J);
    stab = chain_sum_b(group_sum(stab)) / (float)a.E / (float)a.L / (float)J;
    if (l == 0) {
        float* lp = a.loss_part + ((int64_t)x.net * co.tiles + co.tile) * 2;
        lp[0] = x.j_lo > 0 ? lp[0] + beh : beh;
        lp[1] = x.j_lo > 0 ? lp[1] + stab : stab;
    }
}

__global__ __launch_bounds__(D2_THREADS, 2) void beh_dec_fwd2_kernel(IplanBehArgs a) {
    IPLAN_DYN_LDS(smem);
    D2Ctx x;
    x.s_gi = smem;
    x.s_hx = x.s_gi + D2_GI;
    x.s_ux = x.s_hx + D2_HX;
    x.s_yx = x.s_ux + D2_UX;
    int* s_cnt = reinterpret_cast<int*>(x.s_yx + D2_YX);
    x.s_scale = reinterpret_cast<float*>(s_cnt + D2_CNT_INTS);
    if (threadIdx.x < D2_CNT_INTS) s_cnt[threadIdx.x] = 0;
    const int w = uniform_i(wave_id()), role = w >> 2;
    x.q = w & 3;
    x.l = lane_id(); x.n = x.l & 15; x.g = x.l >> 4; x.net = (int)blockIdx.y;
    x.PD = a.dec_params + (int64_t)x.net * a.dec_s_net;
    x.Lw = a.L;
    DecTile c[D2_TILES];
#pragma unroll
    for (int k = 0; k < D2_TILES; ++k) dec_tile(a, c[k], (int)blockIdx.x * D2_TILES + k);
    x.J = c[0].J;
    x.j_lo = imax(a.fwd_j_lo, 0);
    x.j_hi = a.fwd_j_hi > 0 ? imin(a.fwd_j_hi, x.J) : x.J;
    x.steps = (x.j_hi - x.j_lo) * x.Lw;
    x.steps_per_chain = (int64_t)x.J * x.Lw;
    x.cgs = (uint32_t)(x.steps_per_chain * 1024);
    x.YL = 16 * ((a.d + 3) / 4);
    x.hcnt = s_cnt + 0; x.ucnt = s_cnt + 1; x.ycnt = s_cnt + 12; x.rcnt = s_cnt + 16; x.gcnt = s_cnt + 4 + x.q; x.bcnt = s_cnt + 8 + x.q;
    x.n_live = 0;
    bool fast = true;
#pragma unroll
    for (int k = 0; k < D2_TILES; ++k) { x.n_live += c[k].live ? 1 : 0; fast = fast && c[k].full; }
    for (int jj = x.j_lo + w; jj < x.j_hi; jj += D2_THREADS / 64) {
        const float sc = (float)(a.d * a.N) / (window_mask_sum(a, x.net, jj) + BEPS);
        if (x.l == 0) x.s_scale[jj - x.j_lo] = sc;
    }
    __syncthreads();
    const bool fastu = uniform_i(fast ? 1 : 0) != 0;
    if (role == 0) {
        if (a.fwd_skip_act) { if (fastu) d2_recurrent<true, false>(a, x, c); else d2_recurrent<false, false>(a, x, c); }
        else { if (fastu) d2_recurrent<true, true>(a, x, c); else d2_recurrent<false, true>(a, x, c); }
    } else if (x.q == 0) {
        if (fastu) d2_input<true, true>(a, x, c); else d2_input<false, true>(a, x, c);
    } else {
        if (fastu) d2_input<true, false>(a, x, c); else d2_input<false, false>(a, x, c);
    }
}

constexpr int B2_TILES = 3, B2_THREADS = 512;
constexpr int B2_GX = B2_TILES * 8 * 3 * 256;
constexpr int B2_LX = 2 * B2_TILES * 4 * 256;
constexpr int B2_DY = 4 * B2_TILES * 256;
constexpr int B2_TURN = 8 * 2 * 256;
constexpr int B2_CNT_INTS = 16;
constexpr int B2_LDS_FLOATS = B2_GX + B2_LX + B2_DY + B2_TURN + B2_CNT_INTS + D2_MAX_WINDOWS;
constexpr int TP_WOUT = 0, TP_BOUT = 1024, TP_WLIN = 1040, TP_BLIN = 2064;
static_assert(IPLAN_BEH_DEC_THIN_PART >= TP_BLIN + 64 && IPLAN_BEH_DEC_THIN_PART % 16 == 0, "dec_thin_part layout");

struct B2Ctx {
    float *s_gx, *s_lx, *s_dy, *s_turn, *s_scale;
    int *gcnt, *rcnt, *lcnt, *ocnt, *dcnt;
    int q, l, n, g, net, J, Lw, j_lo, j_hi, steps, n_live;
    int64_t steps_per_chain;
    uint32_t cgs;
    const float* PD;
};
__device__ __forceinline__ void b2_g_write(const B2Ctx& x, int k, int gate, f32x4 v) {
    bf16x4 p0, p1, p2;
    split_bf3_half(v, p0, p1, p2);
    char* slot = reinterpret_cast<char*>(x.s_gx + ((k * 8 + gate * 2 + (x.q >> 1)) * 3) * 256) + 16 * x.l + 8 * (x.q & 1);
    *reinterpret_cast<bf16x4*>(slot) = p0;
    *reinterpret_cast<bf16x4*>(slot + 1024) = p1;
    *reinterpret_cast<bf16x4*>(slot + 2048) = p2;
}
__device__ __forceinline__ Bf3 b2_g_read(const B2Ctx& x, int k, int chunk) {
    const char* slot = reinterpret_cast<const char*>(x.s_gx + ((k * 8 + chunk) * 3) * 256) + 16 * x.l;
    Bf3 v;
    v.p0 = *reinterpret_cast<const bf16x8*>(slot);
    v.p1 = *reinterpret_cast<const bf16x8*>(slot + 1024);
    v.p2 = *reinterpret_cast<const bf16x8*>(slot + 2048);
    return v;
}
__device__ __forceinline__ f32x4 b2_chunk(const Bf3& W, const Bf3& G, f32x4 acc) {
    acc = mfma_bf16(W.p2, G.p0, acc); acc = mfma_bf16(W.p0, G.p2, acc); acc = mfma_bf16(W.p1, G.p1, acc);
    acc = mfma_bf16(W.p1, G.p0, acc); acc = mfma_bf16(W.p0, G.p1, acc); acc = mfma_bf16(W.p0, G.p0, acc);
    return acc;
}

__device__ __forceinline__ f32x4 b2_outer_acc(const B2Ctx& x, f32x4 P, f32x4 Q, f32x4 acc) {
    const int n = x.n, g = x.g;
    float* t0 = x.s_turn;
    float* t1 = x.s_turn + 256;
    *reinterpret_cast<f32x4*>(&t0[n * 16 + ((4 * g + 4 * (n >> 1)) & 15)]) = P;
    *reinterpret_cast<f32x4*>(&t1[n * 16 + ((4 * g + 4 * (n >> 1)) & 15)]) = Q;
    IPLAN_WAVE_SYNC();
    for (int s4 = 0; s4 < 4; ++s4) {
        const int r = 4 * s4 + g, o = r * 16 + ((n + 4 * (r >> 1)) & 15);
        acc = mfma4(t0[o], t1[o], acc);
    }
    IPLAN_WAVE_SYNC();
    return acc;
}
__device__ __forceinline__ void b2_store_thin(float* part, bool add, f32x4 acc, int row0, int ld, int col0, int n, int g) {
    for (int r = 0; r < 4; ++r) {
        float* p = part + (row0 + 4 * g + r) * ld + col0 + n;
        *p = add ? *p + acc[r] : acc[r];
    }
}

template <bool FAST>
__device__ __forceinline__ void b2_recurrent(const IplanBehArgs& a, const B2Ctx& x, const DecTile (&c)[B2_TILES]) {
    const int q = x.q, l = x.l, g = x.g, net = x.net, Lw = x.Lw, J = x.J;
    const float* Whh = x.PD + a.dec_off[IPLAN_DEC_WHH];
    Bf3 W[6];
    for (int ch = 0; ch < 6; ++ch) W[ch] = wfrag_t_bf3(Whh, DHd, 16 * q, 32 * ch);
    f32x4 woutT;
    {
        const float* Wo = x.PD + a.dec_off[IPLAN_DEC_OUT_W];
        for (int r = 0; r < 4; ++r) woutT[r] = (4 * g + r < a.d) ? Wo[(int64_t)(4 * g + r) * DHd + 16 * q + (l & 15)] : 0.f;
    }
    const float inv_keep = 1.0f / (1.0f - a.drop_p);
    const uint32_t sd_lane = 64u * (uint32_t)x.n + 16u * (uint32_t)g;
    struct StepIn {
        f32x4 r, z, n, hn, hp;
    };
    const char* sdb[B2_TILES];
    char* ddb[B2_TILES];
    f32x4 dhd[B2_TILES], hcur[B2_TILES], dhdir[B2_TILES];
    StepIn cur[B2_TILES];
    const bool thin = a.dec_thin_part != nullptr;
    f32x4 gWout = splat4(0.f), gbout = splat4(0.f);
    auto load_step = [&](int k, int j, int t, StepIn& o) {
        const bool valid = FAST || c[k].valid;
        const uint32_t so = sd_lane + (uint32_t)(((int64_t)j * Lw + t) * 1024);
        const bool first = (j == 0 && t == 0);
        o.r = ld4_raw<FAST>(sdb[k], so + x.cgs * REC_CG(SD_R + 16 * q), valid);
        o.z = ld4_raw<FAST>(sdb[k], so + x.cgs * REC_CG(SD_Z + 16 * q), valid);
        o.n = ld4_raw<FAST>(sdb[k], so + x.cgs * REC_CG(SD_N + 16 * q), valid);
        o.hn = ld4_raw<FAST>(sdb[k], so + x.cgs * REC_CG(SD_HN + 16 * q), valid);
        o.hp = ld4_raw<FAST>(sdb[k], (first ? so : so - 1024u) + x.cgs * REC_CG(SD_H + 16 * q), valid);
    };
#pragma unroll
    for (int k = 0; k < B2_TILES; ++k) {
        sdb[k] = reinterpret_cast<const char*>(a.saved_dec + c[k].trow0 * x.steps_per_chain * SVD);
        ddb[k] = reinterpret_cast<char*>(a.dsave_dec + c[k].trow0 * x.steps_per_chain * DSD);
        dhd[k] = splat4(0.f);
        hcur[k] = splat4(0.f);
        dhdir[k] = splat4(0.f);
        if (!FAST && !c[k].live) continue;
        if (x.j_hi < J && a.dec_carry)
            dhd[k] = *reinterpret_cast<const f32x4*>(a.dec_carry + ((int64_t)net * c[k].tiles + c[k].tile) * 1024 + 256 * q + 4 * l);
        load_step(k, x.j_hi - 1, Lw - 1, cur[k]);
        hcur[k] = ld4<FAST>(sdb[k], sd_lane + (uint32_t)((((int64_t)(x.j_hi - 1)) * Lw + (Lw - 1)) * 1024) + x.cgs * REC_CG(SD_H + 16 * q),
                            FAST || c[k].valid);
    }
    int j = x.j_hi - 1, t = Lw - 1;
    for (int s = 0; s < x.steps; ++s) {
        const bool first = (j == 0 && t == 0);
        const uint32_t dof = sd_lane + (uint32_t)(((int64_t)j * Lw + t) * 1024);
        int jn = j, tn = t - 1;
        if (tn < 0) { tn = Lw - 1; --jn; }
        if (s + 1 >= x.steps) { jn = j; tn = t; }
        d2_wait(x.rcnt, 8 * s);
#pragma unroll
        for (int k = 0; k < B2_TILES; ++k)
            if (FAST || c[k].live) d2_wait(x.dcnt + k, s + 1);
#pragma unroll
        for (int k = 0; k < B2_TILES; ++k) {
            if (!FAST && !c[k].live) continue;
            const bool valid = FAST || c[k].valid;
            StepIn in = cur[k];
            in.hp = zero_unless(!first, in.hp);
            if (!FAST) {
                in.r = zero_unless(valid, in.r); in.z = zero_unless(valid, in.z); in.n = zero_unless(valid, in.n);
                in.hn = zero_unless(valid, in.hn); in.hp = zero_unless(valid, in.hp);
            }
            const f32x4 dy = *(reinterpret_cast<const f32x4*>(x.s_dy + ((s & 3) * B2_TILES + k) * 256) + l);
            const f32x4 da = mma_block(woutT, dy, splat4(0.f));
            const f32x4 km = keep_tile(a, net, j, c[k].row, t, q, valid, c[k].rows);
            f32x4 dht, act;
            for (int i = 0; i < 4; ++i) {
                const float th = tanh_f(hcur[k][i]);
                act[i] = th * (km[i] * inv_keep);
                dht[i] = fmaf(da[i] * km[i] * inv_keep, 1.0f - th * th, dhd[k][i]);
            }
            if (thin) {
                gWout = b2_outer_acc(x, dy, act, gWout);
                if (q == 0) gbout += dy;
            }
            const GruGrads o = gru_gates_bwd(dht, in.r, in.z, in.n, in.hn, in.hp);
            st4<FAST>(ddb[k], dof + x.cgs * REC_CG(DD_DR + 16 * q), valid, o.dr);
            st4<FAST>(ddb[k], dof + x.cgs * REC_CG(DD_DZ + 16 * q), valid, o.dz);
            st4<FAST>(ddb[k], dof + x.cgs * REC_CG(DD_DNI + 16 * q), valid, o.dni);
            st4<FAST>(ddb[k], dof + x.cgs * REC_CG(DD_DNH + 16 * q), valid, o.dnh);
            b2_g_write(x, k, 0, o.dr);
            b2_g_write(x, k, 1, o.dz);
            b2_g_write(x, k, 2, o.dni);
            b2_g_write(x, k, 3, o.dnh);
            dhdir[k] = o.dh_direct;
            hcur[k] = in.hp;
            load_step(k, jn, tn, cur[k]);
        }
        d2_signal(x.gcnt);
        d2_wait(x.gcnt, 4 * (s + 1));
#pragma unroll
        for (int k = 0; k < B2_TILES; ++k) {
            if (!FAST && !c[k].live) continue;
            f32x4 pd = dhdir[k];
            for (int ch = 0; ch < 6; ++ch) pd = b2_chunk(W[ch], b2_g_read(x, k, ch < 4 ? ch : ch + 2), pd);
            dhd[k] = pd;
        }
        d2_signal(x.rcnt);
        if (--t < 0) { t = Lw - 1; --j; }
    }
#pragma unroll
    for (int k = 0; k < B2_TILES; ++k)
        if ((FAST || c[k].live) && x.j_lo > 0 && a.dec_carry)
            *reinterpret_cast<f32x4*>(a.dec_carry + ((int64_t)net * c[k].tiles + c[k].tile) * 1024 + 256 * q + 4 * l) = dhd[k];
    if (thin) {
        float* part = a.dec_thin_part + ((int64_t)net * gridDim.x + blockIdx.x) * IPLAN_BEH_DEC_THIN_PART;
        const bool add = x.j_hi < J;
        b2_store_thin(part + TP_WOUT, add, gWout, 0, DHd, 16 * q, x.n, g);
        if (q == 0)
            for (int r = 0; r < 4; ++r) {
                const float sum = chain_sum_b(gbout[r]);
                if (x.n == 0) part[TP_BOUT + 4 * g + r] = add ? part[TP_BOUT + 4 * g + r] + sum : sum;
            }
    }
}

template <bool FAST>
__device__ __forceinline__ void b2_input(const IplanBehArgs& a, const B2Ctx& x, const DecTile (&c)[B2_TILES]) {
    const int q = x.q, l = x.l, g = x.g, Lw = x.Lw, J = x.J, din = a.d + a.Z;
    const float* Wih = x.PD + a.dec_off[IPLAN_DEC_WIH];
    Bf3 W[6];
    for (int ch = 0; ch < 6; ++ch) W[ch] = wfrag_t_bf3(Wih, DHd, 16 * q, 32 * ch);
    f32x4 wlatT;
    {
        const float* Wl = x.PD + a.dec_off[IPLAN_DEC_LIN_W];
        const int z = l & 15;
        for (int r = 0; r < 4; ++r) wlatT[r] = z < a.Z ? Wl[(int64_t)(16 * q + 4 * g + r) * din + a.d + z] : 0.f;
    }
    const uint32_t sd_lane = 64u * (uint32_t)x.n + 16u * (uint32_t)g;
    const char* sdb[B2_TILES];
    char* ddb[B2_TILES];
    f32x4 u[B2_TILES], xin[B2_TILES], dlat[B2_TILES];
    const bool thin = a.dec_thin_part != nullptr;
    f32x4 gWlin[B2_TILES], gblin = splat4(0.f);
    for (int k = 0; k < B2_TILES; ++k) gWlin[k] = splat4(0.f);
#pragma unroll
    for (int k = 0; k < B2_TILES; ++k) {
        sdb[k] = reinterpret_cast<const char*>(a.saved_dec + c[k].trow0 * x.steps_per_chain * SVD);
        ddb[k] = reinterpret_cast<char*>(a.dsave_dec + c[k].trow0 * x.steps_per_chain * DSD);
        dlat[k] = splat4(0.f);
        u[k] = xin[k] = splat4(0.f);
        if (!FAST && !c[k].live) continue;
        const uint32_t so = sd_lane + (uint32_t)((((int64_t)(x.j_hi - 1)) * Lw + (Lw - 1)) * 1024);
        u[k] = ld4_raw<FAST>(sdb[k], so + x.cgs * REC_CG(SD_U + 16 * q), FAST || c[k].valid);
        xin[k] = ld4_raw<FAST>(sdb[k], so + x.cgs * REC_CG(SD_X), FAST || c[k].valid);
    }
    DecTile co = c[0];
    if (q == 1) co = c[1];
    if (q == 2) co = c[B2_TILES - 1];
    const int ko = q < B2_TILES ? q : 0;
    const bool owner = q < B2_TILES && (FAST || co.live);
    const bool ovalid = FAST || co.valid;
    const char* sdo = reinterpret_cast<const char*>(a.saved_dec + co.trow0 * x.steps_per_chain * SVD);
    char* ddo = reinterpret_cast<char*>(a.dsave_dec + co.trow0 * x.steps_per_chain * DSD);
    char* dl_base = reinterpret_cast<char*>(a.dsave_lat + co.grow0 * J * DSL);
    const uint32_t dl_lane = (uint32_t)((int64_t)co.n * J * DSL * 4) + 16u * (uint32_t)g;
    const float pen = a.penalty / (float)J / (float)(a.E_norm > 0 ? a.E_norm : a.E) / (float)Lw;
    struct YIn {
        f32x4 y, nx, xc;
        float m;
    };
    auto y_fetch = [&](YIn& o, int jj, int tt) {
        const uint32_t so = sd_lane + (uint32_t)(((int64_t)jj * Lw + tt) * 1024);
        o.y = ld4_raw<FAST>(sdo, so + x.cgs * REC_CG(SD_Y), ovalid);
        o.nx = ld_row_raw<FAST>(co.hist, co.hist_lane + (uint32_t)((int64_t)beh_y_step(a, jj, tt) * a.h_s_t * 4), ovalid, a.d, g);
        o.m = *reinterpret_cast<const float*>(co.mask + (ovalid ? co.mask_lane : 0u) + 4u * (uint32_t)beh_m_step(a, jj, tt));
        o.xc = splat4(0.f);
        if (a.penalty != 0.f) {
            const int st = beh_x_step(a, jj, tt);
            o.xc = ld_row_raw<FAST>(co.hist, co.hist_lane + (uint32_t)((int64_t)(st < 0 ? 0 : st) * a.h_s_t * 4), ovalid, a.d, g);
        }
    };
    auto publish_dy = [&](const YIn& in, int jj, int tt, int sidx) {
        const float scale = x.s_scale[jj - x.j_lo];
        f32x4 dy;
        for (int i = 0; i < 4; ++i) {
            float v = 0.f;
            if (ovalid && 4 * g + i < a.d) {
                const float er = in.nx[i] - in.y[i];
                v = -((er > 0.f) ? 1.0f : (er < 0.f ? -1.0f : 0.0f)) * in.m * scale;
            }
            dy[i] = v;
        }
        if (a.penalty != 0.f) {
            const bool has_xc = beh_x_step(a, jj, tt) >= 0;
            float d2 = 0.f;
            f32x4 df;
            for (int i = 0; i < 4; ++i) {
                df[i] = (ovalid && 4 * g + i < a.d) ? (has_xc ? in.xc[i] : 0.f) - in.y[i] : 0.f;
                d2 = fmaf(df[i], df[i], d2);
            }
            const float nrm = sqrtf(group_sum(d2));
            if (ovalid && nrm > a.thres)
                for (int i = 0; i < 4; ++i) dy[i] -= pen * df[i] / nrm;
        }
        *(reinterpret_cast<f32x4*>(x.s_dy + ((sidx & 3) * B2_TILES + ko) * 256) + l) = dy;
        d2_signal(x.dcnt + ko);
        if (!thin) st4<FAST>(ddo, sd_lane + (uint32_t)(((int64_t)jj * Lw + tt) * 1024) + x.cgs * REC_CG(DD_DY), ovalid, dy);
    };
    int j = x.j_hi - 1, t = Lw - 1, w = 0;
    int jy = j, ty = t, sy = 0;
    auto y_prev = [&]() { if (--ty < 0) { ty = Lw - 1; --jy; } };
    YIn yin;
    if (owner) {
        y_fetch(yin, jy, ty);
        publish_dy(yin, jy, ty, sy++);
        if (x.steps > 1) {
            y_prev();
            y_fetch(yin, jy, ty);
            publish_dy(yin, jy, ty, sy++);
        }
        if (x.steps > 2) {
            y_prev();
            y_fetch(yin, jy, ty);
        }
    }
    for (int s = 0; s < x.steps; ++s) {
        const uint32_t dof = sd_lane + (uint32_t)(((int64_t)j * Lw + t) * 1024);
        int jn = j, tn = t - 1;
        if (tn < 0) { tn = Lw - 1; --jn; }
        if (s + 1 >= x.steps) { jn = j; tn = t; }
        d2_wait(x.gcnt, 4 * (s + 1));
        f32x4 duk[B2_TILES];
#pragma unroll
        for (int k = 0; k < B2_TILES; ++k) {
            duk[k] = splat4(0.f);
            if (!FAST && !c[k].live) continue;
            for (int ch = 0; ch < 6; ++ch) duk[k] = b2_chunk(W[ch], b2_g_read(x, k, ch), duk[k]);
        }
        d2_signal(x.rcnt);
#pragma unroll
        for (int k = 0; k < B2_TILES; ++k) {
            if (!FAST && !c[k].live) continue;
            const bool valid = FAST || c[k].valid;
            const f32x4 du = duk[k];
            const f32x4 uu = FAST ? u[k] : zero_unless(valid, u[k]);
            f32x4 dup;
            for (int i = 0; i < 4; ++i) dup[i] = uu[i] > 0.f ? du[i] : 0.f;
            if (thin) {
                gWlin[k] = b2_outer_acc(x, dup, xin[k], gWlin[k]);
                gblin += dup;
            } else {
                st4<FAST>(ddb[k], dof + x.cgs * REC_CG(DD_DU + 16 * q), valid, dup);
            }
            dlat[k] = mma_block(wlatT, dup, dlat[k]);
            const uint32_t sn = sd_lane + (uint32_t)(((int64_t)jn * Lw + tn) * 1024);
            u[k] = ld4_raw<FAST>(sdb[k], sn + x.cgs * REC_CG(SD_U + 16 * q), valid);
            xin[k] = ld4_raw<FAST>(sdb[k], sn + x.cgs * REC_CG(SD_X), valid);
        }
        if (owner && s + 2 < x.steps) {
            publish_dy(yin, jy, ty, sy++);
            if (s + 3 < x.steps) {
                y_prev();
                y_fetch(yin, jy, ty);
            }
        }
        if (t == 0) {
            if (w >= 2) d2_wait(x.ocnt, x.n_live * (w - 1));
            float* lx = x.s_lx + (w & 1) * (B2_TILES * 4 * 256);
#pragma unroll
            for (int k = 0; k < B2_TILES; ++k) {
                if (!FAST && !c[k].live) continue;
                *reinterpret_cast<f32x4*>(lx + (k * 4 + q) * 256 + 4 * l) = dlat[k];
                dlat[k] = splat4(0.f);
            }
            d2_signal(x.lcnt);
            if (owner) {
                d2_wait(x.lcnt, 4 * (w + 1));
                const float* p = lx + ko * 4 * 256 + 4 * l;
                const f32x4 sum = (*reinterpret_cast<const f32x4*>(p) + *reinterpret_cast<const f32x4*>(p + 256)) +
                                  (*reinterpret_cast<const f32x4*>(p + 512) + *reinterpret_cast<const f32x4*>(p + 768));
                d2_signal(x.ocnt);
                st4<FAST>(dl_base, dl_lane + (uint32_t)j * (uint32_t)(DSL * 4), ovalid, sum);
            }
            ++w;
        }
        if (--t < 0) { t = Lw - 1; --j; }
    }
    if (thin) {
        float* part = a.dec_thin_part + ((int64_t)x.net * gridDim.x + blockIdx.x) * IPLAN_BEH_DEC_THIN_PART;
        const bool add = x.j_hi < J;
        b2_store_thin(part + TP_WLIN, add, (gWlin[0] + gWlin[1]) + gWlin[B2_TILES - 1], 16 * q, 16, 0, x.n, g);
        for (int r = 0; r < 4; ++r) {
            const float sum = chain_sum_b(gblin[r]);
            if (x.n == 0) part[TP_BLIN + 16 * q + 4 * g + r] = add ? part[TP_BLIN + 16 * q + 4 * g + r] + sum : sum;
        }
    }
}

__global__ __launch_bounds__(256) void beh_dec_thin_grad_kernel(IplanBehArgs a, int n_wg) {
    const int net = (int)blockIdx.y, din = a.d + a.Z;
    const int idx = (int)(blockIdx.x * blockDim.x + threadIdx.x);
    const int sizes[4] = {a.d * DHd, a.d, DHd * din, DHd};
    const int which_of[4] = {IPLAN_DEC_OUT_W, IPLAN_DEC_OUT_B, IPLAN_DEC_LIN_W, IPLAN_DEC_LIN_B};
    int rem = idx, k = -1;
    for (int i = 0; i < 4; ++i) {
        if (rem < sizes[i]) { k = i; break; }
        rem -= sizes[i];
    }
    if (k < 0) return;
    int src;
    switch (k) {
        case 0: src = TP_WOUT + rem; break;
        case 1: src = TP_BOUT + rem; break;
        case 2: src = TP_WLIN + (rem / din) * 16 + rem % din; break;
        default: src = TP_BLIN + rem; break;
    }
    const float* part = a.dec_thin_part + (int64_t)net * n_wg * IPLAN_BEH_DEC_THIN_PART + src;
    float s = 0.f;
    for (int w = 0; w < n_wg; ++w) s += part[(int64_t)w * IPLAN_BEH_DEC_THIN_PART];
    float* dst = a.dec_grad + (int64_t)net * a.dec_grad_s_net + a.dec_off[which_of[k]] + rem;
    *dst = a.dec_grad_beta != 0.f ? fmaf(a.dec_grad_beta, *dst, s) : s;
}

__global__ __launch_bounds__(B2_THREADS, 2) void beh_dec_bwd2_kernel(IplanBehArgs a) {
    IPLAN_DYN_LDS(smem);
    B2Ctx x;
    x.s_gx = smem;
    x.s_lx = x.s_gx + B2_GX;
    x.s_dy = x.s_lx + B2_LX;
    x.s_turn = x.s_dy + B2_DY + uniform_i(wave_id()) * 512;
    int* s_cnt = reinterpret_cast<int*>(x.s_dy + B2_DY + B2_TURN);
    x.s_scale = reinterpret_cast<float*>(s_cnt + B2_CNT_INTS);
    if (threadIdx.x < B2_CNT_INTS) s_cnt[threadIdx.x] = 0;
    const int w = uniform_i(wave_id()), role = w >> 2;
    x.q = w & 3;
    x.l = lane_id(); x.n = x.l & 15; x.g = x.l >> 4; x.net = (int)blockIdx.y;
    x.PD = a.dec_params + (int64_t)x.net * a.dec_s_net;
    x.Lw = a.L;
    DecTile c[B2_TILES];
#pragma unroll
    for (int k = 0; k < B2_TILES; ++k) dec_tile(a, c[k], (int)blockIdx.x * B2_TILES + k);
    x.J = c[0].J;
    x.j_lo = imax(a.bwd_j_lo, 0);
    x.j_hi = a.bwd_j_hi > 0 ? imin(a.bwd_j_hi, x.J) : x.J;
    x.steps = (x.j_hi - x.j_lo) * x.Lw;
    x.steps_per_chain = (int64_t)x.J * x.Lw;
    x.cgs = (uint32_t)(x.steps_per_chain * 1024);
    x.gcnt = s_cnt + 0; x.rcnt = s_cnt + 1; x.lcnt = s_cnt + 2; x.ocnt = s_cnt + 3; x.dcnt = s_cnt + 4;
    x.n_live = 0;
    bool fast = true;
#pragma unroll
    for (int k = 0; k < B2_TILES; ++k) { x.n_live += c[k].live ? 1 : 0; fast = fast && c[k].full; }
    for (int jj = x.j_lo + w; jj < x.j_hi; jj += B2_THREADS / 64) {
        const float sc = (float)(a.d * a.N) / (window_mask_sum(a, x.net, jj) + BEPS) / (a.hard ? 1.0f : (float)x.J);
        if (x.l == 0) x.s_scale[jj - x.j_lo] = sc;
    }
    __syncthreads();
    const bool fastu = uniform_i(fast ? 1 : 0) != 0;
    if (role == 0) {
        if (fastu) b2_recurrent<true>(a, x, c); else b2_recurrent<false>(a, x, c);
    } else {
        if (fastu) b2_input<true>(a, x, c); else b2_input<false>(a, x, c);
    }
}

static int check_beh(const IplanBehArgs* a, const char* what) {
    if (!a) return fail(IPLAN_EINVAL, "%s: null args", what);
    if (a->n_nets < 1 || a->E < 1 || a->N < 1 || a->L < 1 || (a->hard ? a->T / a->L - 1 : a->T - 1 - a->L) < 1 || a->d < 1 || a->Z < 1 ||
        a->d > 16 || a->Z > 16 || a->d + a->Z > 16)
        return fail(IPLAN_EINVAL, "%s: unsupported dims E=%d N=%d T=%d L=%d d=%d Z=%d", what, a->E, a->N, a->T, a->L, a->d, a->Z);
    if (a->win) {
        if (!a->lat_in || !a->hd_in || !a->pred_out || !a->hd_out || a->T != a->L + 2 || !a->saved_dec)
            return fail(IPLAN_EINVAL, "%s: single-window decoder mode needs lat_in, hd_in, pred_out, hd_out, saved_dec and T == L + 2", what);
    } else if (!a->hist || !a->mask || !a->saved_enc || !a->saved_lat) {
        return fail(IPLAN_EINVAL, "%s: null tensor pointer", what);
    }
    if (!a->enc_params || !a->dec_params || !a->saved_dec)
        return fail(IPLAN_EINVAL, "%s: null tensor pointer", what);
    if (a->drop_p < 0.f || a->drop_p >= 1.f) return fail(IPLAN_EINVAL, "%s: dropout p=%f", what, a->drop_p);
    return IPLAN_OK;
}

}

extern "C" int iplan_beh_fwd(const IplanBehArgs* a, iplan_stream_t stream) {
    using namespace iplan;
    if (int rc = check_beh(a, "iplan_beh_fwd")) return rc;
    if (!a->win && (!a->loss_part || !a->loss)) return fail(IPLAN_EINVAL, "iplan_beh_fwd: loss buffers missing");
    if ((a->fwd_j_lo > 0 || a->fwd_j_hi > 0) && (a->win || !a->enc_carry || !a->dec_carry || a->fwd_j_lo < 0 ||
                                                 (a->fwd_j_hi > 0 && a->fwd_j_hi <= a->fwd_j_lo)))
        return fail(IPLAN_EINVAL, "iplan_beh_fwd: a window range needs enc_carry, dec_carry and 0 <= fwd_j_lo < fwd_j_hi");
    const int tiles = (a->E * a->N + 15) / 16;
    const dim3 grid((unsigned)((tiles + 3) / 4), (unsigned)a->n_nets);
    const dim3 dgrid((unsigned)((tiles + DEC_TILES - 1) / DEC_TILES), (unsigned)a->n_nets);
    const int ph = a->win ? 2 : a->fwd_phase;
    if (ph == 0 || ph == 1) {
        if (getenv("IPLAN_ENC_FP32") == nullptr) hipLaunchKernelGGL(beh_enc_fwd_kernel<true>, grid, dim3(256), 0, (hipStream_t)stream, *a);
        else hipLaunchKernelGGL(beh_enc_fwd_kernel<false>, grid, dim3(256), 0, (hipStream_t)stream, *a);
    }
    const bool v2 = !a->win && a->d <= 8 && (a->hard ? a->T / a->L - 1 : a->T - 1 - a->L) <= D2_MAX_WINDOWS && getenv("IPLAN_DEC_FWD_V1") == nullptr;
    if ((ph == 0 || ph == 2) && v2) {
        const dim3 grid2((unsigned)((tiles + D2_TILES - 1) / D2_TILES), (unsigned)a->n_nets);
        const size_t lds = sizeof(float) * D2_LDS_FLOATS;
#ifndef IPLAN_HOST_EMULATION
        (void)hipFuncSetAttribute(reinterpret_cast<const void*>(beh_dec_fwd2_kernel), hipFuncAttributeMaxDynamicSharedMemorySize, (int)lds);
#endif
        hipLaunchKernelGGL(beh_dec_fwd2_kernel, grid2, dim3(D2_THREADS), lds, (hipStream_t)stream, *a);
    } else if (ph == 0 || ph == 2) {
        const size_t lds = sizeof(float) * (2 * 3 * DHd * DLD + DHd * 24 + 16 * DLD + DEC_FWD_BIAS + DEC_TILES * XF_SLOTS * 256 + 16);
#ifndef IPLAN_HOST_EMULATION
        (void)hipFuncSetAttribute(reinterpret_cast<const void*>(beh_dec_fwd_kernel), hipFuncAttributeMaxDynamicSharedMemorySize, (int)lds);
#endif
        hipLaunchKernelGGL(beh_dec_fwd_kernel, dgrid, dim3(DEC_THREADS), lds, (hipStream_t)stream, *a);
    }
    if (!a->win && (ph == 0 || ph == 3)) hipLaunchKernelGGL(beh_loss_kernel, dim3((unsigned)a->n_nets), dim3(64), 0, (hipStream_t)stream, *a);
    return check_launch("iplan_beh_fwd");
}

#if defined(D2_CLOCKS) && !defined(IPLAN_HOST_EMULATION)
extern "C" int iplan_debug_d2_clocks(long long* out) {
    return hipMemcpyFromSymbol(out, HIP_SYMBOL(iplan::g_d2_clk), 16 * sizeof(long long)) == hipSuccess ? 0 : 1;
}
#endif

extern "C" int iplan_beh_bwd(const IplanBehArgs* a, iplan_stream_t stream) {
    using namespace iplan;
    if (int rc = check_beh(a, "iplan_beh_bwd")) return rc;
    if (a->win) return fail(IPLAN_EINVAL, "iplan_beh_bwd: not available in single-window decoder mode");
    if (!a->dsave_dec || !a->dsave_lat || !a->enc_part || !a->enc_grad)
        return fail(IPLAN_EINVAL, "iplan_beh_bwd: dsave_dec / dsave_lat / enc_part / enc_grad missing");
    if ((a->bwd_j_lo > 0 || a->bwd_j_hi > 0) &&
        (a->bwd_phase == 0 || (a->bwd_phase == 1 && !a->dec_carry) || (a->bwd_phase == 2 && !a->enc_carry) || a->bwd_j_lo < 0 ||
         (a->bwd_j_hi > 0 && a->bwd_j_hi <= a->bwd_j_lo)))
        return fail(IPLAN_EINVAL, "iplan_beh_bwd: a window range needs bwd_phase 1 (+ dec_carry) or 2 (+ enc_carry) and 0 <= bwd_j_lo < bwd_j_hi");
    const int tiles = (a->E * a->N + 15) / 16;
    const dim3 grid((unsigned)((tiles + 3) / 4), (unsigned)a->n_nets);
    const dim3 dgrid((unsigned)((tiles + DEC_TILES - 1) / DEC_TILES), (unsigned)a->n_nets);
    const size_t lds = sizeof(float) * (2 * DHd * (3 * DHd + 8) + DHd * 24 + 16 * DLD + DEC_TILES * XB_SLOTS * 256 + 16);
#ifndef IPLAN_HOST_EMULATION
    (void)hipFuncSetAttribute(reinterpret_cast<const void*>(beh_dec_bwd_kernel), hipFuncAttributeMaxDynamicSharedMemorySize, (int)lds);
#endif
    const int jn_hi = a->bwd_j_hi > 0 ? a->bwd_j_hi : (a->hard ? a->T / a->L - 1 : a->T - 1 - a->L);
    const bool v2 = jn_hi - (a->bwd_j_lo > 0 ? a->bwd_j_lo : 0) <= D2_MAX_WINDOWS && getenv("IPLAN_DEC_BWD_V1") == nullptr;
    if (a->bwd_phase != 2 && v2) {
        const dim3 grid2((unsigned)((tiles + B2_TILES - 1) / B2_TILES), (unsigned)a->n_nets);
        const size_t lds2 = sizeof(float) * B2_LDS_FLOATS;
#ifndef IPLAN_HOST_EMULATION
        (void)hipFuncSetAttribute(reinterpret_cast<const void*>(beh_dec_bwd2_kernel), hipFuncAttributeMaxDynamicSharedMemorySize, (int)lds2);
#endif
        hipLaunchKernelGGL(beh_dec_bwd2_kernel, grid2, dim3(B2_THREADS), lds2, (hipStream_t)stream, *a);
        if (a->dec_thin_part && a->bwd_j_lo <= 0) {
            if (!a->dec_grad) return fail(IPLAN_EINVAL, "iplan_beh_bwd: dec_thin_part needs dec_grad");
            const int p_thin = a->d * DHd + a->d + DHd * (a->d + a->Z) + DHd;
            hipLaunchKernelGGL(beh_dec_thin_grad_kernel, dim3((unsigned)((p_thin + 255) / 256), (unsigned)a->n_nets), dim3(256), 0,
                               (hipStream_t)stream, *a, (int)grid2.x);
        }
    } else if (a->bwd_phase != 2) {
        if (a->dec_thin_part) return fail(IPLAN_EINVAL, "iplan_beh_bwd: dec_thin_part is only supported by the decoder BPTT's second form");
        hipLaunchKernelGGL(beh_dec_bwd_kernel, dgrid, dim3(DEC_THREADS), lds, (hipStream_t)stream, *a);
    }
    if (a->bwd_phase != 1) {
        if (getenv("IPLAN_ENC_FP32") == nullptr) hipLaunchKernelGGL(beh_enc_bwd_kernel<true>, grid, dim3(256), 0, (hipStream_t)stream, *a);
        else hipLaunchKernelGGL(beh_enc_bwd_kernel<false>, grid, dim3(256), 0, (hipStream_t)stream, *a);
        if (a->bwd_j_lo <= 0) {
            const int p_enc = 32 * a->d + 32 + 2 * 96 * 32 + 2 * 96 + a->Z * 32 + a->Z;
            hipLaunchKernelGGL(beh_enc_grad_kernel, dim3((unsigned)((p_enc + 255) / 256), (unsigned)a->n_nets), dim3(256), 0,
                               (hipStream_t)stream, *a);
        }
    }
    return check_launch("iplan_beh_bwd");
}
```

Measured before the change: 92030 env-steps/s.

## Specialize decoder kernels on dropout source and strength-reduce keep-mask addressing

Templates the fwd2/bwd2 decoder kernels on the dropout source (none, seeded hash, explicit flags) and picks the variant on the host, removing per-step runtime branching. Replaces the per-step keep-index recomputation with an incrementally advanced walker, and in backward prefetches explicit keep flags one step ahead. Hoists per-tile store bases and column offsets, stores through address-space-1 pointers, and polls LDS counters through address-space-3 pointers, while pinning some values in scalar registers. It also adds more kernel instantiations (larger code size) and subtle address-walk logic that could introduce indexing bugs.

After: 91390 env-steps/s. About the same (-0.7%).

```diff
diff --git a/iplan_amd/csrc/behavior_learn.hip b/iplan_amd/csrc/behavior_learn.hip
--- a/iplan_amd/csrc/behavior_learn.hip
+++ b/iplan_amd/csrc/behavior_learn.hip
@@ -49,11 +49,47 @@
     return k;
 }
 
+enum { DROP_NONE = 0, DROP_SEEDED = 1, DROP_FLAGS = 2 };
+__host__ __device__ inline int beh_drop_source(const IplanBehArgs& a) { return a.keep ? DROP_FLAGS : (a.drop_p > 0.f ? DROP_SEEDED : DROP_NONE); }
+__device__ __forceinline__ int64_t keep_index(const IplanBehArgs& a, int net, int j, int row, int t, int T, int rows) {
+    return ((((int64_t)net * beh_windows(a) + j) * rows + row) * a.L + t) * DHd + 16 * T + 4 * (lane_id() >> 4);
+}
+struct KeepWalk {
+    int64_t at, window;
+    int64_t tile;
+    uint32_t lane;
+};
+__device__ __forceinline__ KeepWalk keep_walk(const IplanBehArgs& a, int net, int j, int t, int tile0, int T, int rows) {
+    KeepWalk w;
+    w.at = ((((int64_t)net * beh_windows(a) + j) * rows + 16 * (int64_t)tile0) * a.L + t) * DHd + 16 * T;
+    w.window = (int64_t)rows * a.L * DHd;
+    w.tile = (int64_t)16 * a.L * DHd;
+    w.lane = (uint32_t)(DHd * a.L * (lane_id() & 15) + 4 * (lane_id() >> 4));
+    return w;
+}
+struct KeepRaw { uint8_t b[4]; };
+__device__ __forceinline__ KeepRaw keep_fetch(const IplanBehArgs& a, const KeepWalk& w, int k, bool valid) {
+    const uint8_t* p = a.keep + (w.at + k * w.tile) + (valid ? w.lane : 0u);
+    KeepRaw r;
+    for (int q = 0; q < 4; ++q) r.b[q] = p[q];
+    return r;
+}
+__device__ __forceinline__ f32x4 keep_mask(const KeepRaw& r, bool valid) {
+    f32x4 k;
+    for (int q = 0; q < 4; ++q) k[q] = valid ? (float)r.b[q] : 0.f;
+    return k;
+}
+template <int DROP>
+__device__ __forceinline__ f32x4 keep_drawn(const IplanBehArgs& a, const KeepWalk& w, int k, bool valid) {
+    static_assert(DROP == DROP_NONE || DROP == DROP_SEEDED, "explicit flags: keep_fetch / keep_mask");
+    if (!valid) return splat4(0.f);
+    if (DROP == DROP_NONE) return splat4(1.0f);
+    return keep_flags4(a.seed, (uint64_t)(w.at + k * w.tile) + w.lane, a.drop_p);
+}
 __device__ __forceinline__ f32x4 keep_tile(const IplanBehArgs& a, int net, int j, int row, int t, int T, bool valid, int rows) {
-    const int l = lane_id(), g = l >> 4;
-    const int64_t base = ((((int64_t)net * beh_windows(a) + j) * rows + row) * a.L + t) * DHd + 16 * T + 4 * g;
     f32x4 k = splat4(0.f);
     if (!valid) return k;
+    const int64_t base = keep_index(a, net, j, row, t, T, rows);
     if (a.keep) {
         for (int q = 0; q < 4; ++q) k[q] = (float)a.keep[base + q];
     } else if (a.drop_p > 0.f) {
@@ -242,6 +278,16 @@
     int64_t grow0;
     int64_t trow0;
 };
+#ifdef IPLAN_HOST_EMULATION
+__device__ inline int64_t pin_s64(int64_t v) { return v; }
+__device__ inline const float* pin_global(const float* p) { return p; }
+#else
+__device__ __forceinline__ int64_t pin_s64(int64_t v) { asm volatile("" : "+s"(v)); return v; }
+__device__ __forceinline__ const float* pin_global(const float* p) {
+    return (const float*)(const __attribute__((address_space(1))) float*)pin_s64(reinterpret_cast<int64_t>(p));
+}
+#endif
+template <bool PIN = false>
 __device__ __forceinline__ void dec_tile(const IplanBehArgs& a, DecTile& c, int tile) {
     const int l = lane_id();
     c.n = l & 15;
@@ -258,8 +304,10 @@
     c.e = rr / a.N;
     c.ent = rr - c.e * a.N;
     c.J = beh_windows(a);
-    c.hist = reinterpret_cast<const char*>(a.hist ? a.hist + (int64_t)c.net * a.h_s_net : nullptr);
-    c.hist_lane = (uint32_t)(((int64_t)c.e * a.h_s_e + (int64_t)c.ent * a.d) * 4);
+    const float* hist = PIN ? pin_global(a.hist) : a.hist;
+    const int64_t h_s_net = PIN ? pin_s64(a.h_s_net) : a.h_s_net, h_s_e = PIN ? pin_s64(a.h_s_e) : a.h_s_e;
+    c.hist = reinterpret_cast<const char*>(hist ? hist + (int64_t)c.net * h_s_net : nullptr);
+    c.hist_lane = (uint32_t)(((int64_t)c.e * h_s_e + (int64_t)c.ent * a.d) * 4);
     c.mask = reinterpret_cast<const char*>(a.mask ? a.mask + (int64_t)c.net * a.E * a.T : nullptr);
     c.mask_lane = (uint32_t)(c.e * a.T * 4);
     c.grow0 = (int64_t)c.net * c.rows + (int64_t)(c.live ? tile : 0) * 16;
@@ -974,11 +1022,17 @@
 constexpr int D2_UX = D2_HX;
 constexpr int D2_YX = D2_TILES * 2 * 4 * 128;
 constexpr int D2_CNT_INTS = 20;
+constexpr int D2_CNT_Y = 12, D2_CNT_R = 16;
 constexpr int D2_MAX_WINDOWS = 512;
 constexpr int D2_LDS_FLOATS = D2_GI + D2_HX + D2_UX + D2_YX + D2_CNT_INTS + D2_MAX_WINDOWS;
 
 typedef int i32x4 __attribute__((ext_vector_type(4)));
+static_assert(D2_TILES <= 4, "d2_wait4 polls rcnt[D2_TILES] as one 16-byte group of counters");
+static_assert((D2_GI + D2_HX + D2_UX + D2_YX) % 4 == 0 && D2_CNT_Y % 4 == 0 && D2_CNT_R % 4 == 0 && D2_CNT_R + 4 <= D2_CNT_INTS,
+              "the counter block and the groups d2_wait4 polls are 16-byte aligned (the dynamic LDS array is)");
 #ifdef IPLAN_HOST_EMULATION
+typedef const int* D2Cnt4;
+__device__ inline D2Cnt4 d2_cnt4(const int* c) { return c; }
 __device__ inline void d2_signal(int* c) { IPLAN_WAVE_SYNC(); if (lane_id() == 0) *c += 1; }
 __device__ inline void d2_wait(const int* c, int target) { while (*reinterpret_cast<const volatile int*>(c) < target) iplan_emu::yield_(); }
 __device__ inline void d2_wait4(const int* c, int target, int live) {
@@ -998,10 +1052,13 @@
     while (__hip_atomic_load(c, __ATOMIC_RELAXED, __HIP_MEMORY_SCOPE_WORKGROUP) < target) __builtin_amdgcn_s_sleep(1);
     asm volatile("" ::: "memory");
 }
-__device__ __forceinline__ void d2_wait4(const int* c, int target, int live) {
+typedef const __attribute__((address_space(3))) int* D2Cnt4;
+__device__ __forceinline__ D2Cnt4 d2_cnt4(const int* c) { return (D2Cnt4)c; }
+__device__ __forceinline__ void d2_wait4(D2Cnt4 c, int target, int live) {
+    typedef const volatile __attribute__((address_space(3))) i32x4* Group;
     const i32x4 dead = {(live & 1) ? 0 : 0x7fffffff, (live & 2) ? 0 : 0x7fffffff, (live & 4) ? 0 : 0x7fffffff, (live & 8) ? 0 : 0x7fffffff};
     for (;;) {
-        const i32x4 v = *reinterpret_cast<const volatile i32x4*>(c) | dead;
+        const i32x4 v = *(Group)c | dead;
         const int lo = min(min(v[0], v[1]), min(v[2], v[3]));
         if (__builtin_amdgcn_readfirstlane(lo) >= target) break;
         __builtin_amdgcn_s_sleep(1);
@@ -1050,6 +1107,8 @@
 #ifdef IPLAN_HOST_EMULATION
 __device__ inline void d2_gload(float& dst, const char* sbase, uint32_t voff) { dst = *reinterpret_cast<const float*>(sbase + voff); }
 __device__ inline const char* d2_ubase(const char* p) { return p; }
+typedef char* D2Global;
+__device__ inline D2Global d2_ustore_base(char* p) { return p; }
 template <int WINDOW> __device__ inline void d2_landed(float (&)[4], float (&)[4]) {}
 template <int WINDOW> __device__ inline void d2_landed(float (&)[4], float (&)[4], float&) {}
 __device__ inline void d2_drain_vm() {}
@@ -1064,6 +1123,8 @@
     asm volatile("s_nop 4" : "+s"(u));
     return u;
 }
+typedef __attribute__((address_space(1))) char* D2Global;
+__device__ __forceinline__ D2Global d2_ustore_base(char* p) { return (D2Global)const_cast<char*>(d2_ubase(p)); }
 template <int WINDOW> __device__ __forceinline__ void d2_landed(float (&a)[4], float (&b)[4]) {
     asm volatile("s_waitcnt vmcnt(%8)" : "+v"(a[0]), "+v"(a[1]), "+v"(a[2]), "+v"(a[3]), "+v"(b[0]), "+v"(b[1]), "+v"(b[2]), "+v"(b[3]) : "n"(WINDOW) : "memory");
 }
@@ -1076,6 +1137,7 @@
 struct D2Ctx {
     float *s_gi, *s_hx, *s_ux, *s_yx, *s_scale;
     int *hcnt, *ucnt, *ycnt, *rcnt, *gcnt, *bcnt;
+    D2Cnt4 ycnt4, rcnt4;
     int q, l, n, g, net, J, Lw, j_lo, j_hi, steps, YL, n_live;
     int64_t steps_per_chain;
     uint32_t cgs;
@@ -1103,11 +1165,19 @@
 __device__ __forceinline__ char* d2_sd_base(const IplanBehArgs& a, const D2Ctx& x, const DecTile& ct) {
     return reinterpret_cast<char*>(a.saved_dec + ct.trow0 * x.steps_per_chain * SVD);
 }
+template <bool FULL>
+__device__ __forceinline__ void d2_st4(D2Global base, uint32_t off, bool valid, f32x4 v) {
+#ifdef IPLAN_HOST_EMULATION
+    st4<FULL>(base, off, valid, v);
+#else
+    if (FULL || valid) *reinterpret_cast<__attribute__((address_space(1))) f32x4*>(base + off) = v;
+#endif
+}
 __device__ __forceinline__ uint32_t d2_sd_off(const D2Ctx& x, int step) {
     return 64u * (uint32_t)x.n + 16u * (uint32_t)x.g + (uint32_t)((int64_t)step * 1024);
 }
 
-template <bool FAST, bool SAVE_ACT>
+template <bool FAST, bool SAVE_ACT, int DROP>
 __device__ __forceinline__ void d2_recurrent(const IplanBehArgs& a, const D2Ctx& x, const DecTile (&c)[D2_TILES]) {
     const int q = x.q, l = x.l, g = x.g, net = x.net, Lw = x.Lw;
     (void)g;
@@ -1132,10 +1202,16 @@
     int live_mask = 0;
 #pragma unroll
     for (int k = 0; k < D2_TILES; ++k) live_mask |= (FAST || c[k].live) ? (1 << k) : 0;
+    D2Global sdb[D2_TILES];
+#pragma unroll
+    for (int k = 0; k < D2_TILES; ++k) sdb[k] = d2_ustore_base(d2_sd_base(a, x, c[k]));
+    const uint32_t cg_r = x.cgs * REC_CG(SD_R + 16 * q), cg_z = x.cgs * REC_CG(SD_Z + 16 * q), cg_n = x.cgs * REC_CG(SD_N + 16 * q),
+                   cg_hn = x.cgs * REC_CG(SD_HN + 16 * q), cg_h = x.cgs * REC_CG(SD_H + 16 * q), cg_a = x.cgs * REC_CG(SD_A + 16 * q);
     D2_CLK_DECL(8);
     int j = x.j_lo, t = 0;
-    for (int s = 0; s < x.steps; ++s) {
-        const uint32_t so = d2_sd_off(x, j * Lw + t);
+    uint32_t so = d2_sd_off(x, j * Lw);
+    KeepWalk kw = keep_walk(a, net, j, 0, c[0].tile, q, c[0].rows);
+    for (int s = 0; s < x.steps; ++s, so += 1024u) {
         D2_CLK(7);
         d2_wait(x.hcnt, 4 * (s + 1));
         d2_wait(x.gcnt, s + 1);
@@ -1169,29 +1245,33 @@
         for (int k = 0; k < D2_TILES; ++k) {
             if (!FAST && !c[k].live) continue;
             const bool valid = FAST || c[k].valid;
-            char* sdb = d2_sd_base(a, x, c[k]);
+            KeepRaw kr;
+            if (DROP == DROP_FLAGS) kr = keep_fetch(a, kw, k, valid);
             if (!(D2_ABL & 1)) {
-                st4<FAST>(sdb, so + x.cgs * REC_CG(SD_R + 16 * q), valid, o[k].r);
-                st4<FAST>(sdb, so + x.cgs * REC_CG(SD_Z + 16 * q), valid, o[k].z);
-                st4<FAST>(sdb, so + x.cgs * REC_CG(SD_N + 16 * q), valid, o[k].n);
-                st4<FAST>(sdb, so + x.cgs * REC_CG(SD_HN + 16 * q), valid, o[k].hn);
-                st4<FAST>(sdb, so + x.cgs * REC_CG(SD_H + 16 * q), valid, o[k].h);
-            }
-            const f32x4 km = keep_tile(a, net, j, c[k].row, t, q, valid, c[k].rows);
+                d2_st4<FAST>(sdb[k], so + cg_r, valid, o[k].r);
+                d2_st4<FAST>(sdb[k], so + cg_z, valid, o[k].z);
+                d2_st4<FAST>(sdb[k], so + cg_n, valid, o[k].n);
+                d2_st4<FAST>(sdb[k], so + cg_hn, valid, o[k].hn);
+                d2_st4<FAST>(sdb[k], so + cg_h, valid, o[k].h);
+            }
+            f32x4 km;
+            if constexpr (DROP == DROP_FLAGS) km = keep_mask(kr, valid);
+            else km = keep_drawn<DROP>(a, kw, k, valid);
             f32x4 act;
             for (int i = 0; i < 4; ++i) act[i] = tanh_f(o[k].h[i]) * (km[i] * inv_keep);
-            if (SAVE_ACT && !(D2_ABL & 1)) st4<FAST>(sdb, so + x.cgs * REC_CG(SD_A + 16 * q), valid, act);
+            if (SAVE_ACT && !(D2_ABL & 1)) d2_st4<FAST>(sdb[k], so + cg_a, valid, act);
             yp[k] = mma_block(wout, act, bout);
         }
         D2_CLK(3);
-        if (s >= 2) d2_wait4(x.rcnt, s - 1, live_mask);
+        if (s >= 2) d2_wait4(x.rcnt4, s - 1, live_mask);
         D2_CLK(4);
 #pragma unroll
         for (int k = 0; k < D2_TILES; ++k)
             if ((FAST || c[k].live) && l < x.YL) *(reinterpret_cast<f32x4*>(x.s_yx + ((k * 2 + (s & 1)) * 4 + q) * 128) + l) = yp[k];
         d2_signal(x.ycnt + q);
         D2_CLK(5);
-        if (++t == Lw) { t = 0; ++j; }
+        kw.at += DHd;
+        if (++t == Lw) { t = 0; ++j; kw.at += kw.window - (int64_t)Lw * DHd; }
     }
     D2_CLK_OUT(0, 8);
 #pragma unroll
@@ -1245,12 +1325,11 @@
         return r;
     };
     const int ko = q < D2_TILES ? q : 0;
-    DecTile co = c[0];
-    if (q == 1) co = c[1];
-    if (q == 2) co = c[D2_TILES - 1];
+    DecTile co;
+    dec_tile(a, co, (int)blockIdx.x * D2_TILES + ko);
     const bool owner = q < D2_TILES && (FAST || co.live);
     const bool ovalid = FAST || co.valid;
-    const uint32_t xoo = q == 1 ? hl[1] : (q == 2 ? hl[D2_TILES - 1] : hl[0]);
+    const uint32_t xoo = ovalid ? co.hist_lane : 0u;
     const uint32_t vmo = ovalid ? 0xFFFFFFFFu : 0u;
     float beh = 0.f, stab = 0.f, err = 0.f;
     struct YIn { float nx[4], xt[4], m, scale; };
@@ -1262,7 +1341,7 @@
     };
     auto finish_y = [&](int s, int jj, int tt, YIn& in) {
         d2_landed<FAST ? D2_VM_WINDOW : 0>(in.nx, in.xt, in.m);
-        d2_wait4(x.ycnt, s + 1, 15);
+        d2_wait4(x.ycnt4, s + 1, 15);
         f32x4 yq[4];
         for (int i = 0; i < 4; ++i) {
             yq[i] = splat4(0.f);
@@ -1375,6 +1454,7 @@
     }
 }
 
+template <bool SAVE_ACT, int DROP>
 __global__ __launch_bounds__(D2_THREADS, 2) void beh_dec_fwd2_kernel(IplanBehArgs a) {
     IPLAN_DYN_LDS(smem);
     D2Ctx x;
@@ -1400,7 +1480,8 @@
     x.steps_per_chain = (int64_t)x.J * x.Lw;
     x.cgs = (uint32_t)(x.steps_per_chain * 1024);
     x.YL = 16 * ((a.d + 3) / 4);
-    x.hcnt = s_cnt + 0; x.ucnt = s_cnt + 1; x.ycnt = s_cnt + 12; x.rcnt = s_cnt + 16; x.gcnt = s_cnt + 4 + x.q; x.bcnt = s_cnt + 8 + x.q;
+    x.hcnt = s_cnt + 0; x.ucnt = s_cnt + 1; x.ycnt = s_cnt + D2_CNT_Y; x.rcnt = s_cnt + D2_CNT_R; x.gcnt = s_cnt + 4 + x.q; x.bcnt = s_cnt + 8 + x.q;
+    x.ycnt4 = d2_cnt4(x.ycnt); x.rcnt4 = d2_cnt4(x.rcnt);
     x.n_live = 0;
     bool fast = true;
 #pragma unroll
@@ -1412,8 +1493,7 @@
     __syncthreads();
     const bool fastu = uniform_i(fast ? 1 : 0) != 0;
     if (role == 0) {
-        if (a.fwd_skip_act) { if (fastu) d2_recurrent<true, false>(a, x, c); else d2_recurrent<false, false>(a, x, c); }
-        else { if (fastu) d2_recurrent<true, true>(a, x, c); else d2_recurrent<false, true>(a, x, c); }
+        if (fastu) d2_recurrent<true, SAVE_ACT, DROP>(a, x, c); else d2_recurrent<false, SAVE_ACT, DROP>(a, x, c);
     } else if (x.q == 0) {
         if (fastu) d2_input<true, true>(a, x, c); else d2_input<false, true>(a, x, c);
     } else {
@@ -1482,7 +1562,7 @@
     }
 }
 
-template <bool FAST>
+template <bool FAST, int DROP>
 __device__ __forceinline__ void b2_recurrent(const IplanBehArgs& a, const B2Ctx& x, const DecTile (&c)[B2_TILES]) {
     const int q = x.q, l = x.l, g = x.g, net = x.net, Lw = x.Lw, J = x.J;
     const float* Whh = x.PD + a.dec_off[IPLAN_DEC_WHH];
@@ -1529,12 +1609,21 @@
                             FAST || c[k].valid);
     }
     int j = x.j_hi - 1, t = Lw - 1;
+    KeepWalk kw = keep_walk(a, net, j, t, c[0].tile, q, c[0].rows);
+    KeepRaw kr[B2_TILES];
+    if constexpr (DROP == DROP_FLAGS) {
+#pragma unroll
+        for (int k = 0; k < B2_TILES; ++k)
+            if (FAST || c[k].live) kr[k] = keep_fetch(a, kw, k, FAST || c[k].valid);
+    }
     for (int s = 0; s < x.steps; ++s) {
         const bool first = (j == 0 && t == 0);
         const uint32_t dof = sd_lane + (uint32_t)(((int64_t)j * Lw + t) * 1024);
         int jn = j, tn = t - 1;
         if (tn < 0) { tn = Lw - 1; --jn; }
-        if (s + 1 >= x.steps) { jn = j; tn = t; }
+        KeepWalk kn = kw;
+        kn.at -= t == 0 ? kw.window - (int64_t)(Lw - 1) * DHd : (int64_t)DHd;
+        if (s + 1 >= x.steps) { jn = j; tn = t; kn = kw; }
         d2_wait(x.rcnt, 8 * s);
 #pragma unroll
         for (int k = 0; k < B2_TILES; ++k)
@@ -1551,7 +1640,9 @@
             }
             const f32x4 dy = *(reinterpret_cast<const f32x4*>(x.s_dy + ((s & 3) * B2_TILES + k) * 256) + l);
             const f32x4 da = mma_block(woutT, dy, splat4(0.f));
-            const f32x4 km = keep_tile(a, net, j, c[k].row, t, q, valid, c[k].rows);
+            f32x4 km;
+            if constexpr (DROP == DROP_FLAGS) km = keep_mask(kr[k], valid);
+            else km = keep_drawn<DROP>(a, kw, k, valid);
             f32x4 dht, act;
             for (int i = 0; i < 4; ++i) {
                 const float th = tanh_f(hcur[k][i]);
@@ -1574,6 +1665,7 @@
             dhdir[k] = o.dh_direct;
             hcur[k] = in.hp;
             load_step(k, jn, tn, cur[k]);
+            if constexpr (DROP == DROP_FLAGS) kr[k] = keep_fetch(a, kn, k, valid);
         }
         d2_signal(x.gcnt);
         d2_wait(x.gcnt, 4 * (s + 1));
@@ -1585,6 +1677,7 @@
             dhd[k] = pd;
         }
         d2_signal(x.rcnt);
+        kw = kn;
         if (--t < 0) { t = Lw - 1; --j; }
     }
 #pragma unroll
@@ -1633,10 +1726,9 @@
         u[k] = ld4_raw<FAST>(sdb[k], so + x.cgs * REC_CG(SD_U + 16 * q), FAST || c[k].valid);
         xin[k] = ld4_raw<FAST>(sdb[k], so + x.cgs * REC_CG(SD_X), FAST || c[k].valid);
     }
-    DecTile co = c[0];
-    if (q == 1) co = c[1];
-    if (q == 2) co = c[B2_TILES - 1];
     const int ko = q < B2_TILES ? q : 0;
+    DecTile co;
+    dec_tile<true>(a, co, (int)blockIdx.x * B2_TILES + ko);
     const bool owner = q < B2_TILES && (FAST || co.live);
     const bool ovalid = FAST || co.valid;
     const char* sdo = reinterpret_cast<const char*>(a.saved_dec + co.trow0 * x.steps_per_chain * SVD);
@@ -1648,15 +1740,16 @@
         f32x4 y, nx, xc;
         float m;
     };
+    const uint32_t hst4 = (uint32_t)uniform_i((int)(uint32_t)(a.h_s_t * 4));
     auto y_fetch = [&](YIn& o, int jj, int tt) {
         const uint32_t so = sd_lane + (uint32_t)(((int64_t)jj * Lw + tt) * 1024);
         o.y = ld4_raw<FAST>(sdo, so + x.cgs * REC_CG(SD_Y), ovalid);
-        o.nx = ld_row_raw<FAST>(co.hist, co.hist_lane + (uint32_t)((int64_t)beh_y_step(a, jj, tt) * a.h_s_t * 4), ovalid, a.d, g);
+        o.nx = ld_row_raw<FAST>(co.hist, co.hist_lane + (uint32_t)beh_y_step(a, jj, tt) * hst4, ovalid, a.d, g);
         o.m = *reinterpret_cast<const float*>(co.mask + (ovalid ? co.mask_lane : 0u) + 4u * (uint32_t)beh_m_step(a, jj, tt));
         o.xc = splat4(0.f);
         if (a.penalty != 0.f) {
             const int st = beh_x_step(a, jj, tt);
-            o.xc = ld_row_raw<FAST>(co.hist, co.hist_lane + (uint32_t)((int64_t)(st < 0 ? 0 : st) * a.h_s_t * 4), ovalid, a.d, g);
+            o.xc = ld_row_raw<FAST>(co.hist, co.hist_lane + (uint32_t)(st < 0 ? 0 : st) * hst4, ovalid, a.d, g);
         }
     };
     auto publish_dy = [&](const YIn& in, int jj, int tt, int sidx) {
@@ -1801,6 +1894,7 @@
     *dst = a.dec_grad_beta != 0.f ? fmaf(a.dec_grad_beta, *dst, s) : s;
 }
 
+template <int DROP>
 __global__ __launch_bounds__(B2_THREADS, 2) void beh_dec_bwd2_kernel(IplanBehArgs a) {
     IPLAN_DYN_LDS(smem);
     B2Ctx x;
@@ -1818,7 +1912,7 @@
     x.Lw = a.L;
     DecTile c[B2_TILES];
 #pragma unroll
-    for (int k = 0; k < B2_TILES; ++k) dec_tile(a, c[k], (int)blockIdx.x * B2_TILES + k);
+    for (int k = 0; k < B2_TILES; ++k) dec_tile<true>(a, c[k], (int)blockIdx.x * B2_TILES + k);
     x.J = c[0].J;
     x.j_lo = imax(a.bwd_j_lo, 0);
     x.j_hi = a.bwd_j_hi > 0 ? imin(a.bwd_j_hi, x.J) : x.J;
@@ -1837,9 +1931,26 @@
     __syncthreads();
     const bool fastu = uniform_i(fast ? 1 : 0) != 0;
     if (role == 0) {
-        if (fastu) b2_recurrent<true>(a, x, c); else b2_recurrent<false>(a, x, c);
+        if (fastu) b2_recurrent<true, DROP>(a, x, c); else b2_recurrent<false, DROP>(a, x, c);
     } else {
         if (fastu) b2_input<true>(a, x, c); else b2_input<false>(a, x, c);
+    }
+}
+
+typedef void (*BehKernel)(IplanBehArgs);
+static BehKernel dec_fwd2_variant(const IplanBehArgs& a) {
+    const bool act = !a.fwd_skip_act;
+    switch (beh_drop_source(a)) {
+        case DROP_FLAGS: return act ? beh_dec_fwd2_kernel<true, DROP_FLAGS> : beh_dec_fwd2_kernel<false, DROP_FLAGS>;
+        case DROP_SEEDED: return act ? beh_dec_fwd2_kernel<true, DROP_SEEDED> : beh_dec_fwd2_kernel<false, DROP_SEEDED>;
+        default: return act ? beh_dec_fwd2_kernel<true, DROP_NONE> : beh_dec_fwd2_kernel<false, DROP_NONE>;
+    }
+}
+static BehKernel dec_bwd2_variant(const IplanBehArgs& a) {
+    switch (beh_drop_source(a)) {
+        case DROP_FLAGS: return beh_dec_bwd2_kernel<DROP_FLAGS>;
+        case DROP_SEEDED: return beh_dec_bwd2_kernel<DROP_SEEDED>;
+        default: return beh_dec_bwd2_kernel<DROP_NONE>;
     }
 }
 
@@ -1881,10 +1992,11 @@
     if ((ph == 0 || ph == 2) && v2) {
         const dim3 grid2((unsigned)((tiles + D2_TILES - 1) / D2_TILES), (unsigned)a->n_nets);
         const size_t lds = sizeof(float) * D2_LDS_FLOATS;
+        const BehKernel fwd2 = dec_fwd2_variant(*a);
 #ifndef IPLAN_HOST_EMULATION
-        (void)hipFuncSetAttribute(reinterpret_cast<const void*>(beh_dec_fwd2_kernel), hipFuncAttributeMaxDynamicSharedMemorySize, (int)lds);
+        (void)hipFuncSetAttribute(reinterpret_cast<const void*>(fwd2), hipFuncAttributeMaxDynamicSharedMemorySize, (int)lds);
 #endif
-        hipLaunchKernelGGL(beh_dec_fwd2_kernel, grid2, dim3(D2_THREADS), lds, (hipStream_t)stream, *a);
+        hipLaunchKernelGGL(fwd2, grid2, dim3(D2_THREADS), lds, (hipStream_t)stream, *a);
     } else if (ph == 0 || ph == 2) {
         const size_t lds = sizeof(float) * (2 * 3 * DHd * DLD + DHd * 24 + 16 * DLD + DEC_FWD_BIAS + DEC_TILES * XF_SLOTS * 256 + 16);
 #ifndef IPLAN_HOST_EMULATION
@@ -1924,10 +2036,11 @@
     if (a->bwd_phase != 2 && v2) {
         const dim3 grid2((unsigned)((tiles + B2_TILES - 1) / B2_TILES), (unsigned)a->n_nets);
         const size_t lds2 = sizeof(float) * B2_LDS_FLOATS;
+        const BehKernel bwd2 = dec_bwd2_variant(*a);
 #ifndef IPLAN_HOST_EMULATION
-        (void)hipFuncSetAttribute(reinterpret_cast<const void*>(beh_dec_bwd2_kernel), hipFuncAttributeMaxDynamicSharedMemorySize, (int)lds2);
+        (void)hipFuncSetAttribute(reinterpret_cast<const void*>(bwd2), hipFuncAttributeMaxDynamicSharedMemorySize, (int)lds2);
 #endif
-        hipLaunchKernelGGL(beh_dec_bwd2_kernel, grid2, dim3(B2_THREADS), lds2, (hipStream_t)stream, *a);
+        hipLaunchKernelGGL(bwd2, grid2, dim3(B2_THREADS), lds2, (hipStream_t)stream, *a);
         if (a->dec_thin_part && a->bwd_j_lo <= 0) {
             if (!a->dec_grad) return fail(IPLAN_EINVAL, "iplan_beh_bwd: dec_thin_part needs dec_grad");
             const int p_thin = a->d * DHd + a->d + DHd * (a->d + a->Z) + DHd;
```
